# Mattdl/CLsurvey

Hardware: AMD Instinct MI355X
Metric: images/sec (train+importance pass), EWC small_VGG9 Tiny-ImageNet task batch (higher is better)
Workload: dtype f32 (bf16x6 split operands on the conv fwd/bwd-data matrix products, fp32 accumulate); 1 GPU; EWC small_VGG9_cl_128_128, Tiny-ImageNet shapes (3x64x64, 20 classes), batch 200: train step + Fisher step (BASELINE configs[1]); batch=200, parallelism=1 GPU

## Files before the change

### clsurvey_amd/_lib.py

```python
import ctypes as C
import os

_HERE = os.path.dirname(os.path.abspath(__file__))
LIB_PATH = os.path.join(_HERE, "libclhip.so")

_p = C.c_void_p
_i = C.c_int
_f = C.c_float
_z = C.c_size_t
_l = C.c_long


class HatParam(C.Structure):
    _fields_ = [("theta", _p), ("grad", _p), ("buf", _p), ("mask_back", _p), ("n", _z), ("is_emb", _i), ("reserved", _i)]


class HatGateJob(C.Structure):
    _fields_ = [("emb_row", _p), ("gate", _p), ("mask_pre", _p), ("n", _i), ("reserved", _i)]


class HatLayer(C.Structure):
    _fields_ = [("w", _p), ("gate_in", _p), ("out", _p), ("K", _z), ("C", _z), ("R", _z)]


class HatWgradJob(C.Structure):
    _fields_ = [("g", _p), ("w", _p), ("gate_in", _p), ("dgate_in", _p), ("K", _i), ("C", _i), ("R", _i), ("reserved", _i)]


class HatEmbJob(C.Structure):
    _fields_ = [("dgate", _p), ("gate", _p), ("mask_pre", _p), ("demb", _p), ("n", _i), ("rows", _i), ("t", _i), ("reserved", _i)]


class PathnetLayer(C.Structure):
    _fields_ = [("w_off", _l), ("b_off", _l), ("pw_off", _l), ("pb_off", _l), ("mod_stride", _l), ("c_out", _i), ("c_in", _i),
                ("R", _i), ("n_out", _i), ("n_in", _i), ("Kp", _i), ("Cp", _i), ("M", _i), ("path", _i * 8),
                ("trainable", C.c_ulonglong)]


class IcarlClass(C.Structure):
    _fields_ = [("row_begin", _i), ("row_end", _i), ("k", _i), ("out_off", _i)]


class LayerDesc(C.Structure):
    _fields_ = [("type", _i), ("cin", _i), ("cout", _i), ("relu", _i), ("pool", _i),
                ("w_off", _l), ("b_off", _l), ("ksize", _i), ("stride", _i), ("pad", _i), ("pool_k", _i), ("pool_s", _i),
                ("bn", _i), ("bn_w_off", _l), ("bn_b_off", _l), ("has_drop", _i)]


SIGNATURES = {
    "clhip_version": (_i, []),
    "clhip_arch": (C.c_char_p, []),
    "clhip_conv3x3_fwd": (_i, [_p, _p, _p, _p, _i, _i, _i, _i, _i, _i, _p]),
    "clhip_conv3x3_relu_pool_fwd": (_i, [_p, _p, _p, _p, _p, _i, _i, _i, _i, _i, _p]),
    "clhip_conv3x3_bwd_weight_unpool": (_i, [_p, _p, _p, _p, _p, _i, _i, _i, _i, _i, _p, _z, _p]),
    "clhip_conv3x3_bwd_data": (_i, [_p, _p, _p, _p, _i, _i, _i, _i, _i, _p]),
    "clhip_conv3x3_bwd_data_unpool": (_i, [_p, _p, _p, _p, _p, _i, _i, _i, _i, _i, _p]),
    "clhip_conv3x3_bwd_weight_ws": (_z, [_i, _i, _i, _i, _i]),
    "clhip_conv3x3_bwd_weight": (_i, [_p, _p, _p, _p, _i, _i, _i, _i, _i, _p, _z, _p]),
    "clhip_conv3x3_bwd_weight_slabs": (_i, [_p, _p, _p, _i, _i, _i, _i, _i, _p, _z, C.POINTER(_i), _p]),
    "clhip_conv3x3_bwd_weight_reduce": (_i, [_p, _p, _p, _i, _i, _i, _p]),
    "clhip_conv3x3_wino_ws": (_z, [_i, _i]),
    "clhip_conv3x3_wino_fwd": (_i, [_p, _p, _p, _p, _p, _i, _i, _i, _i, _i, _i, _p, _z, _p]),
    "clhip_conv3x3_wino_bwd_data": (_i, [_p, _p, _p, _p, _p, _i, _i, _i, _i, _i, _p, _z, _p]),
    "clhip_conv5x5_bs_ws": (_z, [_i, _i]),
    "clhip_conv5x5_bs_fwd": (_i, [_p, _p, _p, _p, _i, _i, _i, _i, _i, _i, _p, _z, _p]),
    "clhip_conv5x5_bs_bwd_data": (_i, [_p, _p, _p, _p, _i, _i, _i, _i, _i, _p, _z, _p]),
    "clhip_conv3x3_bs_ws": (_z, [_i, _i]),
    "clhip_conv3x3_bs_fwd": (_i, [_p, _p, _p, _p, _p, _i, _i, _i, _i, _i, _i, _p, _z, _p]),
    "clhip_conv3x3_bs_bwd_data": (_i, [_p, _p, _p, _p, _p, _i, _i, _i, _i, _i, _p, _z, _p]),
    "clhip_conv3x3_wino_bwd_weight_ws": (_z, [_i, _i, _i, _i, _i]),
    "clhip_conv3x3_wino_bwd_weight": (_i, [_p, _p, _p, _p, _p, _i, _i, _i, _i, _i, _p, _z, _p]),
    "clhip_conv3x3_wino_bwd_ws": (_z, [_i, _i, _i, _i, _i]),
    "clhip_conv3x3_wino_bwd": (_i, [_p, _p, _p, _p, _p, _p, _p, _p, _i, _i, _i, _i, _i, _p, _z, _p]),
    "clhip_maxpool2_fwd": (_i, [_p, _p, _p, _i, _i, _i, _p]),
    "clhip_maxpool2_bwd": (_i, [_p, _p, _p, _i, _i, _i, _p]),
    "clhip_fc_ws": (_z, [_i, _i, _i]),
    "clhip_fc_fwd": (_i, [_p, _p, _p, _p, _i, _i, _i, _i, _p, _z, _p]),
    "clhip_fc_bwd_data": (_i, [_p, _p, _p, _p, _i, _i, _i, _p, _z, _p]),
    "clhip_fc_bwd_weight": (_i, [_p, _p, _p, _p, _i, _i, _i, _p, _z, _p]),
    "clhip_relu_bwd": (_i, [_p, _p, _p, _z, _p]),
    "clhip_softmax_ce": (_i, [_p, _p, _i, _i, _i, _p, _p, _p, _p]),
    "clhip_mse_zero_sum": (_i, [_p, _z, _p, _p, _p]),
    "clhip_reg_sgd_step": (_i, [_p, _p, _p, _p, _p, _z, _f, _f, _f, _f, _i, _p]),
    "clhip_fisher_accum": (_i, [_p, _p, _z, _f, _p]),
    "clhip_mas_accum": (_i, [_p, _p, _z, _f, _f, _p]),
    "clhip_si_step": (_i, [_p, _p, _p, _p, _p, _p, _z, _f, _f, _f, _f, _i, _p]),
    "clhip_si_consolidate": (_i, [_p, _p, _p, _p, _z, _f, _p]),
    "clhip_maxpool_fwd": (_i, [_p, _p, _p, _i, _i, _i, _i, _i, _p]),
    "clhip_maxpool_bwd": (_i, [_p, _p, _p, _i, _i, _i, _i, _i, _p]),
    "clhip_conv2d_bwd_weight_ws": (_z, [_i] * 9),
    "clhip_conv2d_fwd": (_i, [_p, _p, _p, _p] + [_i] * 10 + [_p]),
    "clhip_conv2d_bwd_data": (_i, [_p, _p, _p, _p] + [_i] * 9 + [_p]),
    "clhip_conv2d_bwd_weight": (_i, [_p, _p, _p, _p] + [_i] * 9 + [_p, _z, _p]),
    "clhip_conv3x3_bs_bwd_weight_ws": (_z, [_i] * 5),
    "clhip_conv3x3_bs_bwd_weight": (_i, [_p] * 5 + [_i] * 5 + [_p, _z, _p]),
    "clhip_conv5x5_bs_bwd_weight_ws": (_z, [_i] * 5),
    "clhip_conv5x5_bs_bwd_weight": (_i, [_p] * 4 + [_i] * 5 + [_p, _z, _p]),
    "clhip_conv2d_s2d_ws": (_z, [_i] * 8),
    "clhip_conv2d_s2d_fwd": (_i, [_p, _p, _p, _p] + [_i] * 9 + [_p, _z, _p]),
    "clhip_conv2d_s2d_bwd_weight": (_i, [_p, _p, _p, _p] + [_i] * 8 + [_p, _z, _p]),
    "clhip_imm_merge": (_i, [_p, _p, _p, _i, _z, _p, _p]),
    "clhip_lwf_loss": (_i, [_p, _p, _p, _p, _i, _i, _i, _i, _f, _f, _i, _p, _p, _p, _p]),
    "clhip_packnet_finetune_mask": (_i, [_p, _z, _i, _p]),
    "clhip_packnet_kth_ws": (_z, []),
    "clhip_packnet_kth_abs": (_i, [_p, _p, _z, _i, _z, _p, _p, _z, _p]),
    "clhip_packnet_prune": (_i, [_p, _p, _z, _i, _p, _p]),
    "clhip_mask_grad_zero": (_i, [_p, _p, _z, _i, _p]),
    "clhip_mask_weight_zero": (_i, [_p, _p, _z, _i, _i, _p]),
    "clhip_packnet_sgd_step": (_i, [_p, _p, _p, _p, _z, _i, _f, _f, _f, _i, _p]),
    "clhip_hat_gate": (_i, [_p, _i, _f, _p, _p]),
    "clhip_hat_scale_weight": (_i, [_p, _p, _p, _z, _z, _z, _p]),
    "clhip_hat_weight_grad": (_i, [_p, _p, _p, _p, _p, _i, _i, _i, _p]),
    "clhip_hat_emb_grad": (_i, [_p, _p, _p, _i, _f, _f, _p, _p]),
    "clhip_hat_reg_sums": (_i, [_p, _p, _i, _p, _p]),
    "clhip_hat_backmask": (_i, [_p, _p, _p, _z, _z, _z, _p]),
    "clhip_hat_sgd_ws": (_z, []),
    "clhip_hat_sgd_step": (_i, [_p, _p, _p, _p, _z, _f, _f, _f, _i, _i, _f, _f, _f, _f, _i, _p, _z, _p]),
    "clhip_clamp": (_i, [_p, _z, _f, _f, _p]),
    "clhip_hat_sgd_multi_ws": (_z, [_i]),
    "clhip_hat_sgd_step_multi": (_i, [_p, _i, _f, _f, _f, _i, _f, _f, _f, _f, _f, _i, _p, _z, _p]),
    "clhip_hat_gates_multi": (_i, [_p, _i, _f, _p, _p]),
    "clhip_hat_scale_weights_multi": (_i, [_p, _i, _p]),
    "clhip_hat_weight_grads_multi": (_i, [_p, _i, _p]),
    "clhip_hat_emb_grads_multi": (_i, [_p, _i, _f, _f, _f, _p, _p]),
    "clhip_pathnet_ws": (_z, [_p, _i]),
    "clhip_pathnet_pack_multi": (_i, [_p, _i, _p, _z, _p, _z, _p]),
    "clhip_pathnet_fold_grads_multi": (_i, [_p, _i, _p, _z, _p, _z, _p, _z, _p]),
    "clhip_pathnet_sgd_step": (_i, [_p, _i, _p, _p, _p, _z, _f, _f, _f, _f, _i, _p, _z, _p]),
    "clhip_softmax_ce_slice": (_i, [_p, _p, _i, _i, _i, _i, _i, _p, _p, _p, _p]),
    "clhip_net_loss_step_slice": (_i, [_p, _p, _p, _p, _p, _i, _i, _i, _i, _p, _p, _p, _p, _p]),
    "clhip_axpy": (_i, [_p, _p, _z, _f, _i, _p]),
    "clhip_gem_gram_ws": (_z, [_i]),
    "clhip_gem_gram": (_i, [_p, _z, C.POINTER(_i), _i, _z, _p, _p, _z, _p]),
    "clhip_gem_project": (_i, [_p, _z, C.POINTER(_i), C.POINTER(_f), _i, _p, _p, _z, _p]),
    "clhip_gem_qp": (_i, [_p, _i, C.c_double, C.c_double, _p, _p, _p]),
    "clhip_gem_project_dev": (_i, [_p, _z, C.POINTER(_i), _p, _p, _i, _p, _p, _z, _p]),
    "clhip_gem_gram_wide_ws": (_z, [_i]),
    "clhip_gem_gram_wide": (_i, [_p, _z, C.POINTER(_i), _i, _z, _p, _p, _z, _p]),
    "clhip_gem_qp_wide_ws": (_z, [_i]),
    "clhip_gem_qp_wide": (_i, [_p, _i, C.c_double, C.c_double, _p, _p, _p, _z, _p]),
    "clhip_gem_project_wide": (_i, [_p, _z, C.POINTER(_i), C.POINTER(_f), _i, _p, _p, _z, _p]),
    "clhip_gem_project_dev_wide": (_i, [_p, _z, C.POINTER(_i), _p, _p, _i, _p, _p, _z, _p]),
    "clhip_net_create": (_i, [C.POINTER(LayerDesc), _i, _i, _i, _i, _i, C.POINTER(_p)]),
    "clhip_net_set_dropout": (_i, [_p, _i, _p, _l]),
    "clhip_net_set_bn": (_i, [_p, _i, _p, _p, _f, _f]),
    "clhip_net_set_training": (_i, [_p, _i]),
    "clhip_net_probe": (_i, [_p, _i]),
    "clhip_net_probe_read": (_i, [_p, C.POINTER(_f), C.POINTER(_i)]),
    "clhip_net_layer_input": (_i, [_p, _i, _p, _p]),
    "clhip_net_layer_pool_idx": (_i, [_p, _i, _p, _p]),
    "clhip_net_prepared_weights": (_i, [_p, _p, _p]),
    "clhip_net_edge_grid_count": (_i, [_p]),
    "clhip_net_layer_paths": (_i, [_p, _i]),
    "clhip_net_probe_kind": (_i, [_p, _i, _i]),
    "clhip_net_set_input_grad": (_i, [_p, _i, _p]),
    "clhip_sigmoid_fwd": (_i, [_p, _p, _z, _p]),
    "clhip_sigmoid_bwd": (_i, [_p, _p, _p, _z, _p]),
    "clhip_mse_mean": (_i, [_p, _p, _z, _f, _p, _p, _p]),
    "clhip_adadelta_step": (_i, [_p, _p, _p, _p, _z, _f, _f, _f, _f, _p]),
    "clhip_bn_ws": (_z, [_i]),
    "clhip_bn_fwd": (_i, [_p, _p, _p, _p, _p, _p, _p, _p, _i, _i, _i, _i, _f, _f, _i, _p, _z, _p]),
    "clhip_bn_bwd": (_i, [_p, _p, _p, _p, _p, _p, _p, _p, _p, _i, _i, _i, _i, _i, _p, _z, _p]),
    "clhip_net_destroy": (None, [_p]),
    "clhip_net_workspace_bytes": (_z, [_p]),
    "clhip_net_num_classes": (_i, [_p]),
    "clhip_net_forward": (_i, [_p, _p, _p, _i, _p, _p, _p]),
    "clhip_net_backward": (_i, [_p, _p, _p, _p, _i, _p, _p, _p]),
    "clhip_net_loss_step": (_i, [_p, _p, _p, _p, _p, _i, _i, _p, _p, _p, _p, _p]),
    "clhip_rehearsal_assemble": (_i, [_p, _p, _i, _z, _p, _p, _l, _l, _i, _p, _i, _p, _p, _p]),
    "clhip_rehearsal_assemble_crop_flip": (_i, [_p, _p, _i, _i, _i, _i, _i, _i, _p, _l, _p, _p, _p, _l, _l, _i, _p, _p, _i, _p, _p, _p]),
    "clhip_rehearsal_assemble_resized_crop_flip": (_i, [_p, _p, _i, _i, _i, _i, _i, _i, _p, _l, _p, _p, _p, _l, _l, _i, _p, _p, _i, _p, _p, _p]),
    "clhip_loss_segments": (_i, [_p, _p, _p, _i, _i, _i, _p, _i, _f, _p, _p, _p, _p]),
    "clhip_net_loss_step_loss_segments": (_i, [_p, _p, _p, _p, _p, _p, _i, _i, _p, _i, _f, _p, _p, _p, _p, _p]),
    "clhip_gather_tasks": (_i, [_p, _i, _z, _p, _i, _p, _p, _p]),
    "clhip_slice_argmax_count": (_i, [_p, _i, _i, _p, _i, _p, _p, _p, _p, _p]),
    "clhip_gather_tasks_crop_flip": (_i, [_p, _i, _i, _i, _i, _i, _i, _p, _p, _i, _p, _p, _p]),
    "clhip_gather_tasks_resized_crop_flip": (_i, [_p, _i, _i, _i, _i, _i, _i, _p, _p, _i, _p, _p, _p]),
    "clhip_gather_tasks_u8": (_i, [_p, _i, _i, _z, _p, _p, _i, _p, _p, _p]),
    "clhip_gather_tasks_crop_flip_u8": (_i, [_p, _i, _i, _i, _i, _i, _i, _p, _p, _p, _i, _p, _p, _p]),
    "clhip_gather_tasks_resized_crop_flip_u8": (_i, [_p, _i, _i, _i, _i, _i, _i, _p, _p, _p, _i, _p, _p, _p]),
    "clhip_rehearsal_assemble_crop_flip_u8": (_i, [_p, _p, _i, _i, _i, _i, _i, _i, _p, _p, _l, _p, _p, _p, _l, _l, _i, _p, _p, _i, _p, _p, _p]),
    "clhip_rehearsal_assemble_resized_crop_flip_u8": (_i, [_p, _p, _i, _i, _i, _i, _i, _i, _p, _p, _l, _p, _p, _p, _l, _l, _i, _p, _p, _i, _p, _p, _p]),
    "clhip_icarl_herd": (_i, [_p, _l, _i, _p, C.POINTER(IcarlClass), _i, _p, _l, _p]),
    "clhip_icarl_herd_wide_ws": (_z, [_i, _i]),
    "clhip_icarl_herd_wide": (_i, [_p, _l, _i, _p, C.POINTER(IcarlClass), _i, _p, _l, _p, _z, _p]),
    "clhip_icarl_nme": (_i, [_p, _p, _i, _i, _i, _i, _i, _p, _p]),
    "clhip_icarl_assemble_crop_flip": (_i, [_p, _p, _i, _i, _i, _i, _i, _i, _p, _l, _p, _p, _i, _p, _i, _p, _p, _p, _p]),
    "clhip_icarl_assemble_crop_flip_u8": (_i, [_p, _p, _i, _i, _i, _i, _i, _i, _p, _p, _l, _p, _p, _i, _p, _i, _p, _p, _p, _p]),
    "clhip_icarl_assemble_resized_crop_flip": (_i, [_p, _p, _i, _i, _i, _i, _i, _i, _p, _l, _p, _p, _i, _p, _i, _p, _p, _p, _p]),
    "clhip_icarl_assemble_resized_crop_flip_u8": (_i, [_p, _p, _i, _i, _i, _i, _i, _i, _p, _p, _l, _p, _p, _i, _p, _i, _p, _p, _p, _p]),
}

_lib = None


def lib():
    global _lib
    if _lib is None:
        path = os.environ.get("CLHIP_LIB", LIB_PATH)
        if not os.path.exists(path):
            raise RuntimeError(
                "clsurvey_amd: %s not found. Build it with `python clsurvey_amd/build.py` "
                "(hipcc --offload-arch=gfx950). There is no CPU fallback." % path)
        import torch
        bundled = os.path.join(os.path.dirname(torch.__file__), "lib", "libamdhip64.so")
        if os.path.exists(bundled):
            C.CDLL(bundled, mode=C.RTLD_GLOBAL)
        h = C.CDLL(path)
        for name, (res, args) in SIGNATURES.items():
            fn = getattr(h, name)
            fn.restype = res
            fn.argtypes = args
        _lib = h
    return _lib


class ClhipError(RuntimeError):
    pass


def check(rc, what):
    if rc != 0:
        if rc > 0:
            raise ClhipError("%s: HIP error %d" % (what, rc))
        names = {-1: "CLHIP_EINVAL", -2: "CLHIP_ENOSPC", -3: "CLHIP_ENOTSUP"}
        raise ClhipError("%s: %s" % (what, names.get(rc, rc)))
```

### clsurvey_amd/csrc/bsconv.hip

```cpp
#include "common.hpp"
#include "bs_weight.hpp"
#include <cstdlib>

#ifndef BS_ABL
#define BS_ABL 0
#endif

namespace {

constexpr int BS_WT_JOBS = 24;
struct BsWtJobs { int n; int pad; clhip_wino_wt j[BS_WT_JOBS]; int first[BS_WT_JOBS + 1]; };

__global__ __launch_bounds__(256) void bs_weight_multi_kernel(BsWtJobs J) {
    int jb = 0;
    for (int i = 1; i < J.n; ++i) jb = ((int)blockIdx.x >= J.first[i]) ? i : jb;
    bs_weight_block(J.j[jb], (int)blockIdx.x - J.first[jb], (int)threadIdx.x);
}

template <int RW_, int RH_, int NI_, int WAVES_M_, int WM_, int WN_, int KS_ = 3>
struct BsGeo {
    static constexpr int RW = RW_, RH = RH_, NI = NI_, WAVES_M = WAVES_M_, WAVES_N = 4 / WAVES_M_, WM = WM_, WN = WN_;
    static constexpr int KS = KS_, HP = KS_ / 2, TAPS = KS_ * KS_;
    static constexpr int BM = RW * RH * NI;
    static_assert(BM == 32 * WAVES_M * WM, "pixels per block = M tiles of the waves");
    static_assert(32 * WAVES_N * WN == BS_BN, "64 output channels per block");
    static constexpr int MTW = RW >= 16 ? 16 : 8, MTH = 32 / MTW;
    static_assert(RW % MTW == 0 && RH % MTH == 0, "whole M tiles");
    static constexpr int MT_PER_ROW = RW / MTW, MT_PER_IMG = MT_PER_ROW * (RH / MTH);
    static constexpr int IPR = RW == 8 ? 2 : 1;
    static_assert(NI % IPR == 0, "image pairs");
    static constexpr int HW_ = RW + 2 * HP, HR = RH + 2 * HP;
    static constexpr int P = (IPR * HW_ + 7) / 16 * 16 + 8;
    static_assert(P >= IPR * HW_ && P % 16 == 8, "pitch");
    static constexpr int ROWS = (NI / IPR) * HR;
    static constexpr int PLANE_SLOTS = (ROWS - 1) * P + IPR * HW_;
    static constexpr int PLANE_BYTES = PLANE_SLOTS * 16;
    static constexpr int BUF_BYTES = 6 * PLANE_BYTES;
    static constexpr int NHALO = NI * HR * HW_;
    static constexpr int ITEMS = 2 * NHALO;
    static constexpr int ROUNDS = (ITEMS + 255) / 256;
    static_assert(ROUNDS * 256 - ITEMS <= ITEMS, "the last round wraps at most once");
    static constexpr int TPR = WM < MT_PER_ROW ? WM : MT_PER_ROW;
    static_assert(WM % TPR == 0 && MT_PER_ROW % TPR == 0 && MT_PER_IMG % WM == 0, "a wave's tiles form a rectangle inside one image");
    static constexpr int RGW = TPR * MTW, RGH = 32 * WM / RGW;
    static constexpr int TS = 32 * WM + 4;
    static_assert(4 * 32 * TS * 4 <= 2 * BUF_BYTES, "transposition buffers fit the staging LDS");
};

template <class G, int MODE, bool UNPOOL>
__device__ __forceinline__ void bs_conv_body(
    unsigned char* __restrict__ lds, const int b, const float* __restrict__ in, const clhip_u32x4* __restrict__ wimg,
    const float* __restrict__ bias, const float* __restrict__ mask_src, float* __restrict__ out, uint8_t* __restrict__ pool_idx, int N,
    int Cin, int Cout, int H, int W, int relu, int tiles_x, int tiles_y, int npb) {
    constexpr int RW = G::RW, RH = G::RH, NI = G::NI, WM = G::WM, WN = G::WN, P = G::P, HR = G::HR, HW_ = G::HW_;
    constexpr int ROUNDS = G::ROUNDS;

    const int tid = threadIdx.x, lane = tid & 63, wave = tid >> 6;
    const int kts = (Cout + BS_BN - 1) / BS_BN;
    const int kt = (b >> 3) % kts, pb = (b / (8 * kts)) * 8 + (b & 7);
    if (pb >= npb) return;
    const int tx = pb % tiles_x, ty = (pb / tiles_x) % tiles_y, grp = pb / (tiles_x * tiles_y);
    const int n0 = grp * NI, y0 = ty * RH, x0 = tx * RW;
    const int n_chunks = Cin / BS_CK;
    const int IH = UNPOOL ? H >> 1 : H, IW = UNPOOL ? W >> 1 : W;
    const int plane_in = IH * IW;

    const float* in_blk = in + (size_t)n0 * Cin * plane_in;
    const __amdgpu_buffer_rsrc_t rs_x = clhip_rsrc(in_blk, (size_t)(N - n0) * Cin * plane_in * sizeof(float));
    const __amdgpu_buffer_rsrc_t rs_i = clhip_rsrc(UNPOOL ? pool_idx + (size_t)n0 * Cin * plane_in : pool_idx,
                                                   UNPOOL ? (size_t)(N - n0) * Cin * plane_in : 0);
    const int n_nt = (Cout + 31) / 32;
    constexpr int TAPS = G::TAPS, KS = G::KS;
    const __amdgpu_buffer_rsrc_t rs_w = clhip_rsrc(wimg, (size_t)n_nt * n_chunks * 3 * TAPS * 1024);

    int xoff[ROUNDS], lw[ROUNDS], pos[ROUNDS];
#pragma unroll
    for (int r = 0; r < ROUNDS; ++r) {
        const int it_ = r * 256 + tid, it = it_ < G::ITEMS ? it_ : it_ - G::ITEMS;
        const int h = it >= G::NHALO ? 1 : 0, p = it - h * G::NHALO;
        const int ni = p / (HR * HW_), rem = p - ni * (HR * HW_), hy = rem / HW_, hx = rem - hy * HW_;
        const int gy = y0 + hy - G::HP, gx = x0 + hx - G::HP, n = n0 + ni;
        const bool ok = n < N && gy >= 0 && gy < H && gx >= 0 && gx < W;
        const int e = UNPOOL ? (gy >> 1) * IW + (gx >> 1) : gy * IW + gx;
        xoff[r] = ok ? (ni * Cin + 8 * h) * plane_in + e : CLHIP_OOB;
// ... 238 lines not shown
                if (MODE == 0) {
                    y00 += bv; y01 += bv; y10 += bv; y11 += bv;
                    if (relu) { y00 = fmaxf(y00, 0.f); y01 = fmaxf(y01, 0.f); y10 = fmaxf(y10, 0.f); y11 = fmaxf(y11, 0.f); }
                    if (pool) {
                        float mx = y00; int am = 0;
                        if (y01 > mx) { mx = y01; am = 1; }
                        if (y10 > mx) { mx = y10; am = 2; }
                        if (y11 > mx) { mx = y11; am = 3; }
                        if (relu && !(mx > 0.f)) am = CLHIP_POOL_DEAD;
                        if (ok && (!(BS_ABL & 16) || mx == 12345.678f)) {
                            const size_t o = ((size_t)n * Cout + k) * OH * OW + (size_t)(oh >> 1) * OW + (ow >> 1);
                            out[o] = mx;
                            pool_idx[o] = (uint8_t)am;
                        }
                        continue;
                    }
                }
                if (!ok || ((BS_ABL & 16) && y00 != 12345.678f)) continue;
                const size_t o = ((size_t)n * Cout + k) * chw + (size_t)oh * W + ow;
                if (odd) {
                    const bool row1 = oh + 1 < H, col1 = ow + 1 < W;
                    if (MODE == 1 && mask_src) {
                        y00 = mask_src[o] > 0.f ? y00 : 0.f;
                        if (col1) y01 = mask_src[o + 1] > 0.f ? y01 : 0.f;
                        if (row1) y10 = mask_src[o + W] > 0.f ? y10 : 0.f;
                        if (row1 && col1) y11 = mask_src[o + W + 1] > 0.f ? y11 : 0.f;
                    }
                    out[o] = y00;
                    if (col1) out[o + 1] = y01;
                    if (row1) out[o + W] = y10;
                    if (row1 && col1) out[o + W + 1] = y11;
                } else {
                    if (MODE == 1 && mask_src) {
                        const float2 m0 = *reinterpret_cast<const float2*>(mask_src + o), m1 = *reinterpret_cast<const float2*>(mask_src + o + W);
                        y00 = m0.x > 0.f ? y00 : 0.f; y01 = m0.y > 0.f ? y01 : 0.f;
                        y10 = m1.x > 0.f ? y10 : 0.f; y11 = m1.y > 0.f ? y11 : 0.f;
                    }
                    *reinterpret_cast<float2*>(out + o) = make_float2(y00, y01);
                    *reinterpret_cast<float2*>(out + o + W) = make_float2(y10, y11);
                }
            }
        }
    }
    }
}

template <class G, bool UNPOOL>
constexpr int bs_blocks_per_cu() {
    return (3 * 2 * G::BUF_BYTES <= 160 * 1024 && (G::RW == 32 || (!UNPOOL && G::KS == 3))) ? 3 : 2;
}

template <class G, int MODE, bool UNPOOL>
__global__ __launch_bounds__(256, (bs_blocks_per_cu<G, UNPOOL>())) void bs_conv_kernel(
    const float* __restrict__ in, const clhip_u32x4* __restrict__ wimg, const float* __restrict__ bias,
    const float* __restrict__ mask_src, float* __restrict__ out, uint8_t* __restrict__ pool_idx, int N, int Cin, int Cout, int H,
    int W, int relu, int tiles_x, int tiles_y, int npb) {
    __shared__ __attribute__((aligned(16))) unsigned char lds[2 * G::BUF_BYTES];
    bs_conv_body<G, MODE, UNPOOL>(lds, (int)blockIdx.x, in, wimg, bias, mask_src, out, pool_idx, N, Cin, Cout, H, W, relu, tiles_x, tiles_y, npb);
}

template <class GA, class GB, int MODE, bool UNPOOL>
__global__ __launch_bounds__(256, (bs_blocks_per_cu<GA, UNPOOL>() < bs_blocks_per_cu<GB, UNPOOL>() ? bs_blocks_per_cu<GA, UNPOOL>()
                                                                                                  : bs_blocks_per_cu<GB, UNPOOL>()))
void bs_conv_mixed_kernel(const float* __restrict__ in, const clhip_u32x4* __restrict__ wimg, const float* __restrict__ bias,
                          const float* __restrict__ mask_src, float* __restrict__ out, uint8_t* __restrict__ pool_idx, int N, int Cin,
                          int Cout, int H, int W, int relu, int blocks_a, int NA, int tiles_xa, int tiles_ya, int npb_a, int tiles_xb,
                          int tiles_yb, int npb_b) {
    constexpr int LB = 2 * (GA::BUF_BYTES > GB::BUF_BYTES ? GA::BUF_BYTES : GB::BUF_BYTES);
    __shared__ __attribute__((aligned(16))) unsigned char lds[LB];
    const int b = (int)blockIdx.x;
    if (b < blocks_a) {
        bs_conv_body<GA, MODE, UNPOOL>(lds, b, in, wimg, bias, mask_src, out, pool_idx, NA, Cin, Cout, H, W, relu, tiles_xa, tiles_ya, npb_a);
    } else {
        const size_t in_img = (size_t)Cin * (UNPOOL ? (size_t)(H >> 1) * (W >> 1) : (size_t)H * W);
        const bool pool = MODE == 0 && pool_idx != nullptr;
        const size_t out_img = (size_t)Cout * (pool ? (size_t)(H >> 1) * (W >> 1) : (size_t)H * W);
        uint8_t* idx_b = pool_idx ? pool_idx + (size_t)NA * (UNPOOL ? in_img : out_img) : nullptr;
        bs_conv_body<GB, MODE, UNPOOL>(lds, b - blocks_a, in + (size_t)NA * in_img, wimg, bias,
                                       mask_src ? mask_src + (size_t)NA * Cout * H * W : nullptr, out + (size_t)NA * out_img, idx_b, N - NA,
                                       Cin, Cout, H, W, relu, tiles_xb, tiles_yb, npb_b);
    }
}


static int bs_env_int(const char* name, int dflt) {
    const char* e = getenv(name);
    return e && e[0] ? atoi(e) : dflt;
}

template <class G, int MODE, bool UNPOOL>
int bs_launch_geo(const float* in, const clhip_u32x4* wimg, const float* bias, const float* mask_src, float* out, uint8_t* pool_idx,
                  int N, int Cin, int Cout, int H, int W, int relu, hipStream_t s) {
    const int tiles_x = (W + G::RW - 1) / G::RW, tiles_y = (H + G::RH - 1) / G::RH, groups = (N + G::NI - 1) / G::NI;
    const long long npb = (long long)tiles_x * tiles_y * groups;
    const int kts = (Cout + BS_BN - 1) / BS_BN;
    const long long blocks = (npb + 7) / 8 * 8 * kts;
    if (blocks <= 0 || blocks > 0x7fffffffLL) return CLHIP_EINVAL;
    hipLaunchKernelGGL((bs_conv_kernel<G, MODE, UNPOOL>), dim3((unsigned)blocks), dim3(256), 0, s, in, wimg, bias, mask_src, out,
                       pool_idx, N, Cin, Cout, H, W, relu, tiles_x, tiles_y, (int)npb);
    CLHIP_LAUNCH_CHECK();
    return 0;
}

template <int MODE, bool UNPOOL>
int bs_launch_mixed32(const float* in, const clhip_u32x4* wimg, const float* bias, const float* mask_src, float* out, uint8_t* pool_idx,
                      int N, int Cin, int Cout, int H, int W, int relu, hipStream_t s, bool* taken) {
    using GA = BsGeo<32, 4, 1, 2, 2, 1>;
    using GB = BsGeo<32, 2, 1, 2, 1, 1>;
    *taken = false;
    static const int on = bs_env_int("CLHIP_BS_MIXED", 1);
    if (!on) return 0;
    const int kts = (Cout + BS_BN - 1) / BS_BN;
    const long long per_img_a = (long long)((W + GA::RW - 1) / GA::RW) * ((H + GA::RH - 1) / GA::RH);
    const long long slots = 256LL * bs_blocks_per_cu<GA, UNPOOL>();
    const long long total = per_img_a * N * kts, rounds = total / slots, rem = total - rounds * slots;
    if (rounds < 1 || rem == 0 || 2 * rem > slots) return 0;
    const long long na = rounds * slots / (per_img_a * kts);
    if (na < 1 || na >= N || na % 8) return 0;
    const int NA = (int)na;
    const int txa = (W + GA::RW - 1) / GA::RW, tya = (H + GA::RH - 1) / GA::RH, txb = (W + GB::RW - 1) / GB::RW, tyb = (H + GB::RH - 1) / GB::RH;
    const long long npb_a = (long long)txa * tya * NA, npb_b = (long long)txb * tyb * (N - NA);
    const long long blocks_a = (npb_a + 7) / 8 * 8 * kts, blocks_b = (npb_b + 7) / 8 * 8 * kts;
    if (blocks_a + blocks_b > 0x7fffffffLL) return 0;
    hipLaunchKernelGGL((bs_conv_mixed_kernel<GA, GB, MODE, UNPOOL>), dim3((unsigned)(blocks_a + blocks_b)), dim3(256), 0, s, in, wimg, bias,
                       mask_src, out, pool_idx, N, Cin, Cout, H, W, relu, (int)blocks_a, NA, txa, tya, (int)npb_a, txb, tyb, (int)npb_b);
    CLHIP_LAUNCH_CHECK();
    *taken = true;
    return 0;
}

template <int MODE, bool UNPOOL>
int bs_launch(const float* in, const clhip_u32x4* wimg, const float* bias, const float* mask_src, float* out, uint8_t* pool_idx,
              int N, int Cin, int Cout, int H, int W, int relu, hipStream_t s) {
    if (W > 16 && !((H | W) & 1)) {
        bool taken = false;
        const int rc = bs_launch_mixed32<MODE, UNPOOL>(in, wimg, bias, mask_src, out, pool_idx, N, Cin, Cout, H, W, relu, s, &taken);
        if (rc || taken) return rc;
    }
#define BS_GO(...) return bs_launch_geo<BsGeo<__VA_ARGS__>, MODE, UNPOOL>(in, wimg, bias, mask_src, out, pool_idx, N, Cin, Cout, H, W, relu, s)
    if (W > 16) BS_GO(32, 4, 1, 2, 2, 1);
    if (W > 8) BS_GO(16, 8, 1, 2, 2, 1);
    BS_GO(8, 8, 2, 2, 2, 1);
#undef BS_GO
}

template <int MODE>
int bs_launch5(const float* in, const clhip_u32x4* wimg, const float* bias, const float* mask_src, float* out, int N, int Cin, int Cout,
               int H, int W, int relu, hipStream_t s) {
    if (W > 16) return bs_launch_geo<BsGeo<32, 4, 1, 2, 2, 1, 5>, MODE, false>(in, wimg, bias, mask_src, out, nullptr, N, Cin, Cout, H, W, relu, s);
    return bs_launch_geo<BsGeo<16, 8, 1, 2, 2, 1, 5>, MODE, false>(in, wimg, bias, mask_src, out, nullptr, N, Cin, Cout, H, W, relu, s);
}

}

bool clhip_internal_bs_ok(int Cin, int Cout, int H, int W) {
    return Cin >= 32 && Cin % 32 == 0 && Cout >= 64 && Cout % 64 == 0 && H >= 4 && W >= 4;
}

bool clhip_internal_bs_index_ok(int Cin, int Cout, int H, int W, int ks) {
    const long long px = (long long)H * W, ni = (ks == 3 && W <= 8) ? 2 : 1;
    const long long img = (long long)((Cout + 31) / 32) * ((Cin + BS_CK - 1) / BS_CK) * 3 * ks * ks * 1024;
    return ni * Cin * px < (1LL << 29) && Cout * px < (1LL << 29) && img <= 0x7fffffffLL;
}

bool clhip_internal_bs_preferred(int Cin, int Cout, int H, int W) {
    static const int mode = bs_env_int("CLHIP_BS", 1);
    if (mode == 0 || !clhip_internal_bs_ok(Cin, Cout, H, W)) return false;
    if (mode == 2) return true;
    const long long px = (long long)H * W;
    return (px >= 1024 && px <= 4096 && Cin <= 128 && Cout <= 128) || (px >= 512 && px < 1024 && Cin >= 256 && Cout >= 256);
}
bool clhip_internal_bs5_preferred(int Cin, int Cout, int H, int W) {
    static const int mode = bs_env_int("CLHIP_BS", 1);
    return mode != 0 && clhip_internal_bs_ok(Cin, Cout, H, W) && W > 8;
}

size_t clhip_internal_bs_ws(int Cin, int Cout) {
    return (size_t)((Cout + 31) / 32) * ((Cin + BS_CK - 1) / BS_CK) * 27 * 1024;
}
size_t clhip_internal_bs5_ws(int Cin, int Cout) {
    return (size_t)((Cout + 31) / 32) * ((Cin + BS_CK - 1) / BS_CK) * 75 * 1024;
}

int clhip_internal_bs_weights(const clhip_wino_wt* jobs, int n, hipStream_t s) {
    if (n <= 0) return 0;
    if (!jobs) return CLHIP_EINVAL;
    for (int base = 0; base < n; base += BS_WT_JOBS) {
        BsWtJobs J;
        J.n = n - base < BS_WT_JOBS ? n - base : BS_WT_JOBS;
        J.pad = 0;
        int blocks = 0;
        for (int i = 0; i < J.n; ++i) {
            const clhip_wino_wt& q = jobs[base + i];
            if (!q.w || !q.U || q.Ko <= 0 || q.Ci <= 0) return CLHIP_EINVAL;
            J.j[i] = q;
            J.first[i] = blocks;
            blocks += bs_weight_blocks(q);
        }
        J.first[J.n] = blocks;
        hipLaunchKernelGGL(bs_weight_multi_kernel, dim3(blocks), dim3(256), 0, s, J);
        CLHIP_LAUNCH_CHECK();
    }
    return 0;
}

int clhip_internal_bs_conv_u(int mode, const float* in, const void* wimg, const float* bias, const float* mask_src, float* out,
                             uint8_t* pool_idx, int unpool, int N, int Cin, int Cout, int H, int W, int relu, hipStream_t s) {
    if (!in || !wimg || !out || N <= 0 || !clhip_internal_bs_ok(Cin, Cout, H, W) || !clhip_internal_bs_index_ok(Cin, Cout, H, W, 3)) return CLHIP_EINVAL;
    if (((H | W) & 1) && (pool_idx || unpool)) return CLHIP_ENOTSUP;
    const clhip_u32x4* img = static_cast<const clhip_u32x4*>(wimg);
    if (mode == 0) return bs_launch<0, false>(in, img, bias, nullptr, out, pool_idx, N, Cin, Cout, H, W, relu, s);
    if (unpool) return bs_launch<1, true>(in, img, nullptr, mask_src, out, pool_idx, N, Cin, Cout, H, W, 0, s);
    return bs_launch<1, false>(in, img, nullptr, mask_src, out, nullptr, N, Cin, Cout, H, W, 0, s);
}

int clhip_internal_bs5_conv_u(int mode, const float* in, const void* wimg, const float* bias, const float* mask_src, float* out, int N,
                              int Cin, int Cout, int H, int W, int relu, hipStream_t s) {
    if (!in || !wimg || !out || N <= 0 || !clhip_internal_bs_ok(Cin, Cout, H, W) || W <= 8 || !clhip_internal_bs_index_ok(Cin, Cout, H, W, 5))
        return CLHIP_EINVAL;
    const clhip_u32x4* img = static_cast<const clhip_u32x4*>(wimg);
    if (mode == 0) return bs_launch5<0>(in, img, bias, nullptr, out, N, Cin, Cout, H, W, relu, s);
    return bs_launch5<1>(in, img, nullptr, mask_src, out, N, Cin, Cout, H, W, 0, s);
}

extern "C" {

size_t clhip_conv5x5_bs_ws(int C, int K) {
    const size_t a = clhip_internal_bs5_ws(C, K), b = clhip_internal_bs5_ws(K, C);
    return a > b ? a : b;
}

int clhip_conv5x5_bs_fwd(const float* x, const float* w, const float* b, float* y, int N, int C, int K, int H, int W, int relu, void* ws,
                         size_t ws_bytes, void* stream) {
    if (N <= 0 || !clhip_internal_bs_ok(C, K, H, W) || W <= 8) return CLHIP_ENOTSUP;
    if (!x || !w || !y || !ws || ws_bytes < clhip_internal_bs5_ws(C, K)) return CLHIP_EINVAL;
    if (!clhip_internal_bs_index_ok(C, K, H, W, 5)) return CLHIP_EINVAL;
    const clhip_wino_wt job{w, static_cast<float*>(ws), K, C, 0, 5};
    const int rc = clhip_internal_bs_weights(&job, 1, as_stream(stream));
    if (rc) return rc;
    return clhip_internal_bs5_conv_u(0, x, ws, b, nullptr, y, N, C, K, H, W, relu, as_stream(stream));
}

int clhip_conv5x5_bs_bwd_data(const float* dy, const float* w, const float* relu_src, float* dx, int N, int C, int K, int H, int W,
                              void* ws, size_t ws_bytes, void* stream) {
    if (N <= 0 || !clhip_internal_bs_ok(K, C, H, W) || W <= 8) return CLHIP_ENOTSUP;
    if (!dy || !w || !dx || !ws || ws_bytes < clhip_internal_bs5_ws(K, C)) return CLHIP_EINVAL;
    if (!clhip_internal_bs_index_ok(K, C, H, W, 5)) return CLHIP_EINVAL;
    const clhip_wino_wt job{w, static_cast<float*>(ws), C, K, 1, 5};
    const int rc = clhip_internal_bs_weights(&job, 1, as_stream(stream));
    if (rc) return rc;
    return clhip_internal_bs5_conv_u(1, dy, ws, nullptr, relu_src, dx, N, K, C, H, W, 0, as_stream(stream));
}

size_t clhip_conv3x3_bs_ws(int C, int K) {
    const size_t a = clhip_internal_bs_ws(C, K), b = clhip_internal_bs_ws(K, C);
    return a > b ? a : b;
}

int clhip_conv3x3_bs_fwd(const float* x, const float* w, const float* b, float* y, uint8_t* idx_u8_or_null, int N, int C, int K, int H,
                         int W, int relu, void* ws, size_t ws_bytes, void* stream) {
    if (N <= 0 || !clhip_internal_bs_ok(C, K, H, W)) return CLHIP_ENOTSUP;
    if (!x || !w || !y || !ws || ws_bytes < clhip_internal_bs_ws(C, K)) return CLHIP_EINVAL;
    if (!clhip_internal_bs_index_ok(C, K, H, W, 3)) return CLHIP_EINVAL;
    if (((H | W) & 1) && idx_u8_or_null) return CLHIP_ENOTSUP;
    const clhip_wino_wt job{w, static_cast<float*>(ws), K, C, 0, 0};
    const int rc = clhip_internal_bs_weights(&job, 1, as_stream(stream));
    if (rc) return rc;
    return clhip_internal_bs_conv_u(0, x, ws, b, nullptr, y, idx_u8_or_null, 0, N, C, K, H, W, relu, as_stream(stream));
}

int clhip_conv3x3_bs_bwd_data(const float* dy, const uint8_t* idx_u8_or_null, const float* w, const float* relu_src, float* dx, int N,
                              int C, int K, int H, int W, void* ws, size_t ws_bytes, void* stream) {
    if (N <= 0 || !clhip_internal_bs_ok(K, C, H, W)) return CLHIP_ENOTSUP;
    if (!dy || !w || !dx || !ws || ws_bytes < clhip_internal_bs_ws(K, C)) return CLHIP_EINVAL;
    if (!clhip_internal_bs_index_ok(K, C, H, W, 3)) return CLHIP_EINVAL;
    if (((H | W) & 1) && idx_u8_or_null) return CLHIP_ENOTSUP;
    const clhip_wino_wt job{w, static_cast<float*>(ws), C, K, 1, 0};
    const int rc = clhip_internal_bs_weights(&job, 1, as_stream(stream));
    if (rc) return rc;
    return clhip_internal_bs_conv_u(1, dy, ws, nullptr, relu_src, dx, const_cast<uint8_t*>(idx_u8_or_null), idx_u8_or_null != nullptr,
                                    N, K, C, H, W, 0, as_stream(stream));
}

}
```

### clsurvey_amd/csrc/common.hpp

```cpp
#pragma once
#include <hip/hip_runtime.h>
#include <stdint.h>
#include <stddef.h>
#include "../../include/clhip.h"

#define CLHIP_LAUNCH_CHECK()                          \
    do {                                              \
        hipError_t e__ = hipGetLastError();           \
        if (e__ != hipSuccess) return (int)e__;       \
    } while (0)

static inline hipStream_t as_stream(void* s) { return reinterpret_cast<hipStream_t>(s); }

static inline bool aligned16(const void* p) { return (reinterpret_cast<uintptr_t>(p) & 15u) == 0; }

static inline bool clhip_conv3x3_dims_ok(int N, int C, int K, int H, int W) {
    if (N <= 0 || C <= 0 || K <= 0 || H <= 0 || W <= 0) return false;
    const long long hw = (long long)H * W;
    if (hw >= (1LL << 23)) return false;
    if (hw * (C + 32LL) >= (1LL << 28) || hw * (K + 32LL) >= (1LL << 28)) return false;
    if ((long long)K * C >= (1LL << 29) / 9) return false;
    return hw * N <= 0x7fffffffLL;
}

// ... 60 lines not shown
    return v;
}
__device__ __forceinline__ float wave_sum(float v) {
#pragma unroll
    for (int o = 32; o > 0; o >>= 1) v += __shfl_xor(v, o, 64);
    return v;
}
__device__ __forceinline__ double wave_sum(double v) {
#pragma unroll
    for (int o = 32; o > 0; o >>= 1) v += __shfl_xor(v, o, 64);
    return v;
}
__device__ __forceinline__ int wave_min(int v) {
#pragma unroll
    for (int o = 32; o > 0; o >>= 1) v = min(v, __shfl_xor(v, o, 64));
    return v;
}

typedef float floatx16 __attribute__((ext_vector_type(16)));
typedef float floatx4 __attribute__((ext_vector_type(4)));

__device__ __forceinline__ int mfma32_row(int r, int lane) { return (r & 3) + 8 * (r >> 2) + 4 * (lane >> 5); }


#define CLHIP_FC_MAX 4
struct clhip_fc_chain {
    int n;
    long w_off[CLHIP_FC_MAX], b_off[CLHIP_FC_MAX];
    int din[CLHIP_FC_MAX], dout[CLHIP_FC_MAX], relu[CLHIP_FC_MAX];
    size_t act_off[CLHIP_FC_MAX], dz_off[CLHIP_FC_MAX];
};
int clhip_internal_fc_chain_ok(const clhip_fc_chain* d);
int clhip_internal_fc_chain_wgrad(const clhip_fc_chain* d, float* grads, const float* x, int N, const float* acts,
                                  const float* dlogits, const float* dz, hipStream_t s);
struct clhip_gemm_args {
    const float* a; const float* b; float* out;
    int M, N, K; long sam, sak, sbk, sbn; int n_tiles, splits, k_per_split;
    const float* bias; const float* mask_src; int relu;
};
int clhip_internal_fc_bwd_data_args(const float* dy, const float* w, const float* relu_src, float* dx, int M, int I, int O,
                                    clhip_gemm_args* args_out);
int clhip_internal_fc_bwd_combo(const clhip_gemm_args* g, int gemm_blocks, const clhip_fc_chain* d, float* grads, const float* x,
                                int N, const float* acts, const float* dlogits, const float* dz, hipStream_t s);

int clhip_internal_fc_tail_ok(const clhip_fc_chain* d);
int clhip_internal_fc_tail(const clhip_fc_chain* d, const float* params, float* acts, int N, const int64_t* labels,
                           int reduction, int col_off, int ncols, float* dlogits, float* fcdz, float* loss_out, double* stats,
                           void* row_scratch, unsigned* counter, int do_loss, int do_bwd, const float* h1_slabs, int live,
                           hipStream_t s);
int clhip_internal_fc_fwd_partial(const float* x, const float* w, int M, int I, int O, void* ws, size_t ws_bytes, int* live,
                                  hipStream_t s);

#define CLHIP_WGRAD_JOBS_MAX 32
struct clhip_wgrad_job { const float* part; float* dw; float* db; int K, C, splits; int taps; };
int clhip_internal_conv3x3_wgrad_partial(const float* x, const float* dy, const uint8_t* unpool_idx, float* dw, float* db, int N,
                                         int C, int K, int H, int W, void* ws, size_t ws_bytes, void* stream, clhip_wgrad_job* job);
int clhip_internal_wgrad_reduce_multi(const clhip_wgrad_job* jobs, int n, hipStream_t s);

bool clhip_internal_convkk_ok(int N, int Cin, int Cout, int H, int W, int R, int S, int stride, int pad);
int clhip_internal_convkk(int mode, const float* in, const float* w, const float* bias, const float* mask_src, float* out, int N,
                          int Cin, int Cout, int H, int W, int relu, hipStream_t s);

struct clhip_wino_wt { const float* w; float* U; int Ko, Ci, mode, pad; };
int clhip_internal_wino_weights(const clhip_wino_wt* jobs, int n, hipStream_t s);
int clhip_internal_weight_images(const clhip_wino_wt* wino_jobs, int n_wino, const clhip_wino_wt* bs_jobs, int n_bs, hipStream_t s);
int clhip_internal_c3w64_pool_weight_images(const float* x, const float* w, const float* b, float* y_pool, uint8_t* idx_u8, int N, int C,
                                            int K, int H, int W, const clhip_wino_wt* wino_jobs, int n_wino, const clhip_wino_wt* bs_jobs,
                                            int n_bs, int wt_first, hipStream_t s);
int clhip_internal_wino_conv_u(int mode, const float* in, const float* U, const float* bias, const float* mask_src, float* out,
                               uint8_t* pool_idx, int unpool, int N, int Cin, int Cout, int H, int W, int relu, hipStream_t s);
bool clhip_internal_wino_ok(int Cin, int Cout, int H, int W);
size_t clhip_internal_wino_ws(int Cin, int Cout);
bool clhip_internal_bs_ok(int Cin, int Cout, int H, int W);
bool clhip_internal_bs_index_ok(int Cin, int Cout, int H, int W, int ks);
bool clhip_internal_bs_preferred(int Cin, int Cout, int H, int W);
bool clhip_internal_bs5_preferred(int Cin, int Cout, int H, int W);
size_t clhip_internal_bs5_ws(int Cin, int Cout);
int clhip_internal_bs5_conv_u(int mode, const float* in, const void* wimg, const float* bias, const float* mask_src, float* out, int N,
                              int Cin, int Cout, int H, int W, int relu, hipStream_t s);
size_t clhip_internal_bs_ws(int Cin, int Cout);
int clhip_internal_bs_weights(const clhip_wino_wt* jobs, int n, hipStream_t s);
int clhip_internal_bs_conv_u(int mode, const float* in, const void* wimg, const float* bias, const float* mask_src, float* out,
                             uint8_t* pool_idx, int unpool, int N, int Cin, int Cout, int H, int W, int relu, hipStream_t s);
bool clhip_internal_bs5_wgrad_ok(int N, int C, int K, int H, int W);
size_t clhip_internal_bs5_wgrad_ws(int N, int C, int K, int H, int W);
int clhip_internal_bs5_wgrad(const float* x, const float* dy, float* dw, float* db, int N, int C, int K, int H, int W, void* ws,
                             size_t ws_bytes, hipStream_t s);
size_t clhip_internal_bs3k_wgrad_ws(int N, int C, int K, int H, int W);
int clhip_internal_bs3k_wgrad(const float* x, const float* dy, float* dw, float* db, int N, int C, int K, int H, int W, void* ws,
                              size_t ws_bytes, hipStream_t s);
bool clhip_internal_bs_wgrad_ok(int C, int K, int H, int W);
bool clhip_internal_bs_wgrad_preferred(int C, int K, int H, int W, int pooled);
size_t clhip_internal_bs_wgrad_ws(int N, int C, int K, int H, int W);
int clhip_internal_bs_wgrad_partial(const float* x, const float* dy, const uint8_t* unpool_idx, float* dw, float* db, int N, int C, int K,
                                    int H, int W, void* ws, size_t ws_bytes, hipStream_t s, clhip_wgrad_job* job);
bool clhip_internal_wino_wgrad_ok(int C, int K, int H, int W);
size_t clhip_internal_wino_wgrad_ws(int N, int C, int K, int H, int W);
int clhip_internal_wino_wgrad_partial(const float* x, const float* dy, const uint8_t* unpool_idx, float* dw, float* db, int N, int C,
                                      int K, int H, int W, void* ws, size_t ws_bytes, hipStream_t s, clhip_wgrad_job* job);
int clhip_internal_wino_pair(const float* dy, const uint8_t* unpool_idx, const float* U, const float* mask_src, float* dx,
                             const float* x, float* dw, float* db, int N, int C, int K, int H, int W, void* ws, size_t ws_bytes,
                             hipStream_t s, clhip_wgrad_job* job);
bool clhip_internal_wino_pair_shape(int N, int C, int K, int H, int W, int pooled);
int clhip_internal_wino_conv(int mode, const float* in, const float* w, const float* bias, const float* mask_src, float* out,
                             uint8_t* pool_idx, int unpool, int N, int Cin, int Cout, int H, int W, int relu, void* ws,
                             size_t ws_bytes, hipStream_t s);
```

### clsurvey_amd/csrc/conv3x3_wgrad.hip

```cpp
#include <cstdlib>
#include "common.hpp"

namespace {

constexpr int KT = 64, CT = 64;

#ifdef CLHIP_TRACE
__device__ unsigned long long* g_wtrace = nullptr;
#define TR_NOW() __builtin_amdgcn_s_memtime()
#endif

template <int TW, int TH>
struct WGeo {
    static constexpr int BP = TW * TH;
    static constexpr int TWP = TW + 2;
    static constexpr int PLANE = (TH + 2) * TWP;
    static constexpr int PLANEP = PLANE | 1;
    static constexpr int LDP = BP + 1;
    static_assert(BP == 64, "stage is 64 pixels");
};

__device__ __forceinline__ void decode_stage(int st, int tiles_w, int tiles_h, int TW, int TH,
                                             int& n, int& h0, int& w0) {
    int tw_i = st % tiles_w;
    int t = st / tiles_w;
    int th_i = t % tiles_h;
    n = t / tiles_h;
    h0 = th_i * TH;
    w0 = tw_i * TW;
}

#ifndef CLHIP_WGRAD_PS_WAVES
#define CLHIP_WGRAD_PS_WAVES 1
#endif
template <int TW, int TH, bool VEC, bool PS, bool UNPOOL = false>
__global__ __launch_bounds__(256, CLHIP_WGRAD_PS_WAVES) void conv3x3_wgrad_kernel(
    const float* __restrict__ x, const float* __restrict__ dy, float* __restrict__ part,
    int N, int C, int K, int H, int W, int tiles_w, int tiles_h,
    int total_stages, int splits, int c_tiles, size_t slab_stride, const uint8_t* __restrict__ unpool_idx) {
    static_assert(!UNPOOL || VEC, "the fused un-pool lives in the 16-byte staging path");
    using G = WGeo<TW, TH>;
    constexpr int KTt = PS ? 32 : 64, CTt = PS ? 32 : 64;
    constexpr int DYS_FLOATS = KTt * G::LDP, XS_FLOATS = CTt * G::PLANEP;
    constexpr int BUF_FLOATS = DYS_FLOATS + XS_FLOATS;
    static_assert(!PS || 2 * BUF_FLOATS >= 9 * 1024 + 3 * 128, "the pixel-split reduction pad lives in the stage buffers");
    __shared__ __attribute__((aligned(16))) float lds[2 * BUF_FLOATS];

    const int tid = threadIdx.x, lane = tid & 63, wave = tid >> 6;
#ifdef CLHIP_TRACE
    const unsigned long long tr_start = TR_NOW();
#endif
    const int wk = PS ? 0 : (wave & 1), wc = PS ? 0 : (wave >> 1);
    const int li = lane & 31, kk = lane >> 5;

    const int split = blockIdx.x % splits;
    const int tile = blockIdx.x / splits;
    const int ct = tile % c_tiles, kt = tile / c_tiles;
    const int k0 = kt * KTt, c0 = ct * CTt;

    const int per = total_stages / splits, extra = total_stages % splits;
    const int st_begin = split * per + min(split, extra);
    const int st_end = st_begin + per + (split < extra ? 1 : 0);

    floatx16 acc[9];
#pragma unroll
    for (int t = 0; t < 9; ++t)
#pragma unroll
        for (int r = 0; r < 16; ++r) acc[t][r] = 0.f;
    double bsum = 0.0;

    const int plane_hw = H * W;
    const int Wp = W >> 1, plane_dy = UNPOOL ? (H >> 1) * Wp : plane_hw;

    constexpr int XROWS = CTt * (TH + 2);
    constexpr int DY_IT = VEC ? (KTt * G::BP / 4) / 256 : KTt * G::BP / 256;
    constexpr int X_ELEMS = CTt * G::PLANE;
    constexpr int XV_ELEMS = XROWS * (TW / 4);
    constexpr int X_IT = VEC ? (XV_ELEMS + 255) / 256 : (X_ELEMS + 255) / 256;
    constexpr int H_IT = VEC ? (XROWS * 2 + 255) / 256 : 0;
    constexpr int NU = DY_IT + X_IT + H_IT;
    float4 dyv[VEC ? DY_IT : 1], xv[VEC ? X_IT : 1];
    float hv[H_IT > 0 ? H_IT : 1];
    float dyr[VEC ? 1 : DY_IT], xr[VEC ? 1 : X_IT];
    int dyoff[DY_IT], dydst[DY_IT], dyrow[DY_IT];
// ... 526 lines not shown
        cur_n = t0 / tiles_h;
    }
    auto load_stage = [&](Stage& S, bool live) {
        const int n = cur_n, h0 = cur_th * 2, w0 = cur_tw * 32;
        if (++cur_tw == tiles_w) { cur_tw = 0; if (++cur_th == tiles_h) { cur_th = 0; ++cur_n; } }
        const int o = __builtin_amdgcn_readfirstlane(live ? (n * K * OH + (h0 >> 1)) * OW + (w0 >> 1) : 0);
        S.gA = clhip_buf_load4(r_dy, live ? dyA_voff : CLHIP_OOB, o * 4);
        S.gB = clhip_buf_load4(r_dy, live ? dyB_voff : CLHIP_OOB, o * 4);
        S.code8 = clhip_buf_load2(r_ix, live ? ix8_voff : CLHIP_OOB, o);
        const int hrow = h0 + wh;
        const unsigned edges = (hrow == 0 ? 1u : 0u) | (hrow + 1 >= H ? 2u : 0u) | (w0 == 0 ? 4u : 0u) | (w0 + 32 >= W ? 8u : 0u);
        const unsigned bad = live ? edge_bits & (unsigned)__builtin_amdgcn_readfirstlane((int)(edges * 0x11111u)) : 0xfffffu;
        const int xo = __builtin_amdgcn_readfirstlane(live ? ((n * C * H + hrow) * W + w0) * 4 : 0);
#pragma unroll
        for (int j = 0; j < 5; ++j)
            S.xr[j] = clhip_buf_load(r_x, (bad & (0xfu << (4 * j))) ? CLHIP_OOB : xe_voff[j], xo);
    };
    auto store_x = [&](const Stage& S, int buf) {
        float* d = xs_w + buf * U3_HALO;
#pragma unroll
        for (int j = 0; j < 5; ++j) d[xe_dst[j]] = S.xr[j];
        float* dd = dy_w + buf * U3_DY;
        *reinterpret_cast<float4*>(dd + dstA) = S.gA;
        *reinterpret_cast<float4*>(dd + dstB) = S.gB;
        *reinterpret_cast<float2*>(dd + dst8) = S.code8;
    };
    auto compute = [&](int buf) {
        const float* row = dy_w + buf * U3_DY + li * U3_DYROW;
        float4 Sg[4];
#pragma unroll
        for (int j = 0; j < 4; ++j) Sg[j] = *reinterpret_cast<const float4*>(row + 4 * j);
        const clhip_u32x4 Scode = *reinterpret_cast<const clhip_u32x4*>(row + 16);
        const float* bp = xs_w + buf * U3_HALO + col_off + kk;
        asm volatile("" : "+a"(acc));
#pragma unroll
        for (int wp = 0; wp < 16; ++wp) {
            const float g = wp & 2 ? (wp & 1 ? Sg[wp >> 2].w : Sg[wp >> 2].z) : (wp & 1 ? Sg[wp >> 2].y : Sg[wp >> 2].x);
            const unsigned word = Scode[wp >> 2];
            const unsigned code = (word >> (8 * (wp & 3))) & 0xffu;
            const float a = code == want ? g : 0.f;
            bsum += (double)a;
            acc = __builtin_amdgcn_mfma_f32_32x32x2f32(a, bp[2 * wp], acc, 0, 0, 0);
        }
        asm volatile("" : "+a"(acc));
    };

    const int n_st = st_end - st_begin;
    if (n_st > 0) {
        Stage SA, SB;
        load_stage(SA, true);
        store_x(SA, 0);
        const int pairs = n_st >> 1;
        for (int i = 0; i < pairs; ++i) {
            load_stage(SB, true);
            compute(0);
            store_x(SB, 1);
            load_stage(SA, 2 * i + 2 < n_st);
            compute(1);
            store_x(SA, 0);
        }
        if (n_st & 1) compute(0);
    }
    bsum += __shfl_xor(bsum, 32, 64);
    if (wh == 1) {
#pragma unroll
        for (int r = 0; r < 16; ++r) red[(wk * 16 + r) * 64 + lane] = acc[r];
        if (kk == 0) red[2048 + wk * 32 + li] = (float)bsum;
    }
    __syncthreads();
    if (wh == 0) {
        float* slab = part + (size_t)split * slab_stride;
        if (li < ncol) {
            const int cc = li / 9, rs = li - cc * 9;
#pragma unroll
            for (int r = 0; r < 16; ++r) {
                const int kr = k0 + wk * 32 + mfma32_row(r, lane);
                if (kr < K) slab[((size_t)rs * K + kr) * C + cc] = acc[r] + red[(wk * 16 + r) * 64 + lane];
            }
        }
        if (kk == 0 && kok) slab[(size_t)9 * K * C + k] = (float)(bsum + (double)red[2048 + wk * 32 + li]);
    }
}

constexpr int RED_EL = 64, RED_J = 16, RED_V = 4;
constexpr int RED_THREADS = RED_EL / RED_V * RED_J;

template <int EL, int J>
__device__ __forceinline__ void wgrad_reduce_block(const float* __restrict__ part, float* __restrict__ dw, float* __restrict__ db,
                                                   int K, int C, int splits, size_t e0, double (*partial)[EL], int T = 9) {
    const size_t kc = (size_t)K * C, nw = (size_t)T * kc, total = nw + K;
    const int v = threadIdx.x % (EL / RED_V), j = threadIdx.x / (EL / RED_V);
    const size_t e = e0 + (size_t)v * RED_V;
    const int q = (splits + J - 1) / J;
    const int s0 = j * q, s1 = min(splits, s0 + q);
    double s[RED_V] = {0.0, 0.0, 0.0, 0.0};
    if ((total & 3) == 0 && (reinterpret_cast<uintptr_t>(part) & 15u) == 0 && e + RED_V <= total) {
#pragma unroll 4
        for (int sp = s0; sp < s1; ++sp) {
            const float4 t = *reinterpret_cast<const float4*>(part + (size_t)sp * total + e);
            s[0] += (double)t.x; s[1] += (double)t.y; s[2] += (double)t.z; s[3] += (double)t.w;
        }
    } else {
        for (int sp = s0; sp < s1; ++sp)
#pragma unroll
            for (int t = 0; t < RED_V; ++t)
                if (e + t < total) s[t] += (double)part[(size_t)sp * total + e + t];
    }
#pragma unroll
    for (int t = 0; t < RED_V; ++t) partial[j][v * RED_V + t] = s[t];
    __syncthreads();
    if (threadIdx.x < EL) {
        const int el = threadIdx.x;
        const size_t ee = e0 + el;
        if (ee < total) {
            double t = 0.0;
#pragma unroll
            for (int jj = 0; jj < J; ++jj) t += partial[jj][el];
            if (ee < nw) {
                const size_t rs = ee / kc, rem = ee - rs * kc;
                dw[rem * T + rs] = (float)t;
            } else if (db) {
                db[ee - nw] = (float)t;
            }
        }
    }
}

template <int EL, int J>
__global__ __launch_bounds__(RED_THREADS) void wgrad_reduce_kernel(const float* __restrict__ part, float* __restrict__ dw,
                                                                   float* __restrict__ db, int K, int C, int splits) {
    __shared__ double partial[J][EL];
    wgrad_reduce_block<EL, J>(part, dw, db, K, C, splits, (size_t)blockIdx.x * EL, partial);
}

struct RedJobs {
    clhip_wgrad_job job[CLHIP_WGRAD_JOBS_MAX];
    unsigned first[CLHIP_WGRAD_JOBS_MAX + 1];
    int n;
};

template <int EL, int JL>
__global__ __launch_bounds__(RED_THREADS) void wgrad_reduce_multi_kernel(RedJobs jobs) {
    __shared__ double partial[JL][EL];
    int ji = 0;
    while (ji + 1 < jobs.n && blockIdx.x >= jobs.first[ji + 1]) ++ji;
    const clhip_wgrad_job J = jobs.job[ji];
    wgrad_reduce_block<EL, JL>(J.part, J.dw, J.db, J.K, J.C, J.splits, (size_t)(blockIdx.x - jobs.first[ji]) * EL, partial, J.taps ? J.taps : 9);
}

struct WPlan {
    int TW, TH, tiles_w, tiles_h, total_stages, splits, k_tiles, c_tiles, group, groups, ps;
    size_t slab, ws_floats;
};

WPlan make_plan(int N, int C, int K, int H, int W) {
    WPlan p;
    if (W > 16) { p.TW = 32; p.TH = 2; }
    else if (W > 8) { p.TW = 16; p.TH = 4; }
    else { p.TW = 8; p.TH = 8; }
    p.tiles_w = (W + p.TW - 1) / p.TW;
    p.tiles_h = (H + p.TH - 1) / p.TH;
    p.total_stages = p.tiles_w * p.tiles_h * N;
    const bool smallc = (C * 9 <= 32);
    p.k_tiles = (K + KT - 1) / KT;
    p.c_tiles = smallc ? 1 : (C + CT - 1) / CT;
    p.ps = 0;
    if (!smallc) {
        const int t64 = p.k_tiles * p.c_tiles;
        const int splits64 = (256 + t64 - 1) / t64;
        if (p.total_stages / (splits64 > 0 ? splits64 : 1) < 8) {
            p.ps = 1;
            p.k_tiles = (K + 31) / 32;
            p.c_tiles = (C + 31) / 32;
        }
    }
    int tiles = p.k_tiles * p.c_tiles;
    int target = smallc ? 1024 : 256;
    if (smallc) {
        static const int t_env = [] { const char* e = getenv("CLHIP_WG_SMALLC_BLOCKS"); return e && e[0] ? atoi(e) : 0; }();
        if (t_env > 0) target = t_env;
    }
    int splits = (target + tiles - 1) / tiles;
    if (splits > p.total_stages) splits = p.total_stages;
    p.slab = (size_t)9 * K * C + K;
    size_t max_splits = ((size_t)64 << 20) / (p.slab * sizeof(float));
    if (max_splits < 1) max_splits = 1;
    if ((size_t)splits > max_splits) splits = (int)max_splits;
    if (splits < 1) splits = 1;
    p.splits = splits;
    int group = 1;
    while (group * group < splits) ++group;
    p.group = group;
    p.groups = (splits + group - 1) / group;
    p.ws_floats = p.slab * (size_t)(splits + p.groups);
    return p;
}

}

extern "C" {

#ifdef CLHIP_TRACE
int clhip_debug_set_wgrad_trace(void* p) {
    unsigned long long* q = static_cast<unsigned long long*>(p);
    return (int)hipMemcpyToSymbol(HIP_SYMBOL(g_wtrace), &q, sizeof(q));
}
#endif

size_t clhip_conv3x3_bwd_weight_ws(int N, int C, int K, int H, int W) {
    if (!clhip_conv3x3_dims_ok(N, C, K, H, W)) return 0;
    return make_plan(N, C, K, H, W).ws_floats * sizeof(float);
}

static int bwd_weight_impl(const float* x, const float* dy, const uint8_t* unpool_idx, float* dw, float* db,
                           int N, int C, int K, int H, int W, void* ws, size_t ws_bytes, void* stream,
                           clhip_wgrad_job* defer = nullptr) {
    if (!x || !dy || !dw || !ws || !clhip_conv3x3_dims_ok(N, C, K, H, W)) return CLHIP_EINVAL;
    if (unpool_idx && ((H & 1) || (W & 1))) return CLHIP_ENOTSUP;
    WPlan p = make_plan(N, C, K, H, W);
    if (ws_bytes < p.ws_floats * sizeof(float)) return CLHIP_ENOSPC;
    hipStream_t s = as_stream(stream);
    float* part = static_cast<float*>(ws);
    const bool smallc = (C * 9 <= 32);
    unsigned grid = (unsigned)(p.k_tiles * p.c_tiles * p.splits);
#define WG_ARGS x, dy, part, N, C, K, H, W, p.tiles_w, p.tiles_h, p.total_stages, p.splits
    if (smallc && unpool_idx && p.TW == 32 && W % 32 == 0 && aligned16(dy) && aligned16(unpool_idx) &&
        (size_t)N * K * H * W < ((size_t)1 << 31) && (size_t)N * C * H * W < ((size_t)1 << 29)) {
        hipLaunchKernelGGL(conv3x3_wgrad_c3_unpool_kernel, dim3(grid), dim3(256), 0, s, WG_ARGS, p.slab, unpool_idx);
    } else if (smallc) {
        if (p.TW == 32) hipLaunchKernelGGL((conv3x3_wgrad_smallc_kernel<32, 2>), dim3(grid), dim3(256), 0, s, WG_ARGS, p.slab, unpool_idx);
        else if (p.TW == 16) hipLaunchKernelGGL((conv3x3_wgrad_smallc_kernel<16, 4>), dim3(grid), dim3(256), 0, s, WG_ARGS, p.slab, unpool_idx);
        else hipLaunchKernelGGL((conv3x3_wgrad_smallc_kernel<8, 8>), dim3(grid), dim3(256), 0, s, WG_ARGS, p.slab, unpool_idx);
    } else {
        const bool vec = (W % 4 == 0) && (W % p.TW == 0) && aligned16(x) && aligned16(dy);
        if (unpool_idx && (!vec || (reinterpret_cast<uintptr_t>(unpool_idx) & 1u))) return CLHIP_ENOTSUP;
#define WG_K(TW_, TH_, VEC_, PS_, UNP_) hipLaunchKernelGGL((conv3x3_wgrad_kernel<TW_, TH_, VEC_, PS_, UNP_>), dim3(grid), dim3(256), 0, s, \
                                                           WG_ARGS, p.c_tiles, p.slab, unpool_idx)
#define WG_LAUNCH1(TW_, TH_, PS_) do { if (unpool_idx) WG_K(TW_, TH_, true, PS_, true); else if (vec) WG_K(TW_, TH_, true, PS_, false); \
                                      else WG_K(TW_, TH_, false, PS_, false); } while (0)
#define WG_LAUNCH(TW_, TH_) do { if (p.ps) WG_LAUNCH1(TW_, TH_, true); else WG_LAUNCH1(TW_, TH_, false); } while (0)
        if (p.TW == 32) WG_LAUNCH(32, 2);
        else if (p.TW == 16) WG_LAUNCH(16, 4);
        else WG_LAUNCH(8, 8);
#undef WG_LAUNCH
#undef WG_LAUNCH1
#undef WG_K
    }
#undef WG_ARGS
    CLHIP_LAUNCH_CHECK();
    if (defer) {
        *defer = clhip_wgrad_job{part, dw, db, K, C, p.splits};
        return 0;
    }
    const unsigned bx = (unsigned)((p.slab + RED_EL - 1) / RED_EL);
    hipLaunchKernelGGL((wgrad_reduce_kernel<RED_EL, RED_J>), dim3(bx), dim3(RED_THREADS), 0, s, part, dw, db, K, C, p.splits);
    CLHIP_LAUNCH_CHECK();
    return 0;
}

int clhip_conv3x3_bwd_weight(const float* x, const float* dy, float* dw, float* db,
                             int N, int C, int K, int H, int W, void* ws, size_t ws_bytes, void* stream) {
    return bwd_weight_impl(x, dy, nullptr, dw, db, N, C, K, H, W, ws, ws_bytes, stream);
}

int clhip_conv3x3_bwd_weight_unpool(const float* x, const float* dy_pool, const uint8_t* idx_u8, float* dw, float* db,
                                    int N, int C, int K, int H, int W, void* ws, size_t ws_bytes, void* stream) {
    if (!idx_u8) return CLHIP_EINVAL;
    return bwd_weight_impl(x, dy_pool, idx_u8, dw, db, N, C, K, H, W, ws, ws_bytes, stream);
}

int clhip_conv3x3_bwd_weight_slabs(const float* x, const float* dy, const uint8_t* idx_u8_or_null, int N, int C, int K, int H,
                                   int W, void* ws, size_t ws_bytes, int* splits_out, void* stream) {
    if (!splits_out || !ws) return CLHIP_EINVAL;
    clhip_wgrad_job job;
    const int rc = bwd_weight_impl(x, dy, idx_u8_or_null, static_cast<float*>(ws), nullptr, N, C, K, H, W, ws, ws_bytes, stream, &job);
    if (rc == 0) *splits_out = job.splits;
    return rc;
}

int clhip_conv3x3_bwd_weight_reduce(const void* ws, float* dw, float* db, int K, int C, int splits, void* stream) {
    if (!ws || !dw || K <= 0 || C <= 0 || splits <= 0) return CLHIP_EINVAL;
    const size_t slab = (size_t)9 * K * C + K;
    const unsigned bx = (unsigned)((slab + RED_EL - 1) / RED_EL);
    hipLaunchKernelGGL((wgrad_reduce_kernel<RED_EL, RED_J>), dim3(bx), dim3(RED_THREADS), 0, as_stream(stream),
                            static_cast<const float*>(ws), dw, db, K, C, splits);
    CLHIP_LAUNCH_CHECK();
    return 0;
}

}

int clhip_internal_conv3x3_wgrad_partial(const float* x, const float* dy, const uint8_t* unpool_idx, float* dw, float* db, int N,
                                         int C, int K, int H, int W, void* ws, size_t ws_bytes, void* stream, clhip_wgrad_job* job) {
    if (!job) return CLHIP_EINVAL;
    return bwd_weight_impl(x, dy, unpool_idx, dw, db, N, C, K, H, W, ws, ws_bytes, stream, job);
}

int clhip_internal_wgrad_reduce_multi(const clhip_wgrad_job* jobs, int n, hipStream_t s) {
    if (n <= 0) return 0;
    if (!jobs || n > CLHIP_WGRAD_JOBS_MAX) return CLHIP_EINVAL;
    RedJobs r;
    r.n = n;
    r.first[0] = 0;
    for (int i = 0; i < n; ++i) {
        r.job[i] = jobs[i];
        const size_t total = (size_t)(jobs[i].taps ? jobs[i].taps : 9) * jobs[i].K * jobs[i].C + jobs[i].K;
        r.first[i + 1] = r.first[i] + (unsigned)((total + RED_EL - 1) / RED_EL);
    }
    for (int i = n; i < CLHIP_WGRAD_JOBS_MAX; ++i) { r.job[i] = clhip_wgrad_job{nullptr, nullptr, nullptr, 0, 0, 0, 0}; r.first[i + 1] = r.first[n]; }
    hipLaunchKernelGGL((wgrad_reduce_multi_kernel<RED_EL, RED_J>), dim3(r.first[n]), dim3(RED_THREADS), 0, s, r);
    CLHIP_LAUNCH_CHECK();
    return 0;
}
```

### clsurvey_amd/csrc/engine.hip

```cpp
#include <vector>
#include <cstdlib>
#include <memory>
#include <new>
#include "common.hpp"

namespace {

enum class Conv : unsigned char {
    None,
    Direct3,
    Wino,
    Bs3,
    Bs5,
    S2d,
    Gemm,
};
enum class Img : unsigned char { None, WinoU, Bs3, Bs5 };
struct WeightImage { Img kind; size_t off; };
enum : unsigned {
    WG_BS = 1,
    WG_WINO = 2,
    WG_3X3 = 4,
    WG_BS5 = 8,
    WG_S2D = 16,
};

struct LayerPlan {
    int type;
    int cin, cout, relu, pool;
    long w_off, b_off;
    int h, w;
    int ks, st, pd;
    int oh, ow;
    int pk, ps;
    int ph, pw;
    bool vgg;
    bool pool22;
    bool fused_pool;
    size_t in_elems, out_elems, pool_elems;
    size_t act_off;
    size_t pool_off;
    size_t idx_off;
    int bn;
    long bn_w_off, bn_b_off;
    size_t z_off;
    size_t stat_off;
    float* rmean; float* rvar; float bn_momentum, bn_eps;
    Conv fwd, bwd;
    WeightImage img_f, img_d;
    unsigned wg;
    size_t wg_off, wg_bytes;
    size_t s2d_off, s2d_bytes;
    size_t scratch_need;
    const float* extra_grad;
    const float* drop;
    long drop_stride;
    int has_drop_buf;
    size_t drop_off;
};

constexpr long long WINO_MIN_UNITS = 640;
constexpr long long WINO16_MIN_UNITS = 384;
constexpr unsigned PROBE_RING = 64;
#ifndef CLHIP_EDGE_GRIDS_DEFAULT
#define CLHIP_EDGE_GRIDS_DEFAULT 1
#endif
#ifndef CLHIP_OVERLAP_DEFAULT
#define CLHIP_OVERLAP_DEFAULT 0
#endif

bool env_starts(const char* name, char c) { const char* e = std::getenv(name); return e && e[0] == c; }
bool wino_enabled() { return !env_starts("CLHIP_WINO", '0'); }
bool bs5_wgrad_enabled() { return !env_starts("CLHIP_BS_WGRAD", '0'); }
bool s2d_enabled() { return env_starts("CLHIP_S2D", '1'); }
bool fc_tail_enabled() { return !env_starts("CLHIP_FC_TAIL", '0'); }
int overlap_mode() { return env_starts("CLHIP_WGRAD_OVERLAP", '1') ? 1 : env_starts("CLHIP_WGRAD_OVERLAP", '2') ? 2 : CLHIP_OVERLAP_DEFAULT; }
int edge_grids_mode() {
    const char* e = std::getenv("CLHIP_EDGE_GRIDS");
    return (e && e[0] >= '0' && e[0] <= '2' && !e[1]) ? e[0] - '0' : CLHIP_EDGE_GRIDS_DEFAULT;
}

struct NetPlan {
    std::vector<LayerPlan> layers;
    int max_batch, in_c, in_h, in_w, n_classes;
    size_t in_elems;
    size_t scratch_bytes;
    size_t wino_bytes;
    size_t off_wino;
    size_t off_s2d;
    int s2d_fresh_n;
    size_t total_bytes;
    size_t off_acts, off_idx, off_g0, off_g1, off_scratch, off_dlogits, off_loss, off_fcdz, off_wg;
    int training = 1;
    int n_wg;
    int fc_first;
    bool fc_fused;
    clhip_fc_chain chain;
    size_t fcdz_floats;
    int probe_layer = -1;
    int probe_kind;
    unsigned probe_count;
    std::vector<hipEvent_t> probe_ev;
    bool fc_tail, no_combo;
    unsigned* tail_counter;
    size_t off_rows;
    int edge_grids;
    unsigned edge_count;
    bool overlap;
    int overlap_mode;
    hipStream_t side;
    std::vector<hipEvent_t> ev_dy, ev_wg;
    ~NetPlan() {
        for (hipEvent_t e : ev_dy) (void)hipEventDestroy(e);
        for (hipEvent_t e : ev_wg) (void)hipEventDestroy(e);
        if (side) (void)hipStreamDestroy(side);
        if (tail_counter) (void)hipFree(tail_counter);
        for (hipEvent_t e : probe_ev) (void)hipEventDestroy(e);
    }
};

inline size_t align_up(size_t v, size_t a) { return (v + a - 1) / a * a; }
inline size_t max_of(size_t a, size_t b) { return a > b ? a : b; }

__global__ void drop_scale_kernel(float* __restrict__ h, const float* __restrict__ mask, long stride, int feat, size_t total) {
    for (size_t i = blockIdx.x * (size_t)blockDim.x + threadIdx.x; i < total; i += (size_t)gridDim.x * blockDim.x) {
        const size_t n = i / feat, f = i - n * feat;
        h[i] *= mask[n * stride + f];
    }
}

__global__ void add_inplace_kernel(float* __restrict__ a, const float* __restrict__ b, size_t n) {
    for (size_t i = blockIdx.x * (size_t)blockDim.x + threadIdx.x; i < n; i += (size_t)gridDim.x * blockDim.x) a[i] += b[i];
}

int add_inplace(float* a, const float* b, size_t n, hipStream_t s) {
    hipLaunchKernelGGL(add_inplace_kernel, dim3(ew_grid(n, 256)), dim3(256), 0, s, a, b, n);
    CLHIP_LAUNCH_CHECK();
    return 0;
}

__global__ void drop_copy_kernel(const float* __restrict__ h, float* __restrict__ out, const float* __restrict__ mask, long stride,
                                 int feat, size_t total) {
    for (size_t i = blockIdx.x * (size_t)blockDim.x + threadIdx.x; i < total; i += (size_t)gridDim.x * blockDim.x) {
        const size_t n = i / feat, f = i - n * feat;
        out[i] = h[i] * mask[n * stride + f];
    }
}

int drop_copy(const float* h, float* out, const float* mask, long stride, size_t feat, int N, hipStream_t s) {
    const size_t total = feat * N;
    hipLaunchKernelGGL(drop_copy_kernel, dim3(ew_grid(total, 256)), dim3(256), 0, s, h, out, mask, stride, (int)feat, total);
    CLHIP_LAUNCH_CHECK();
    return 0;
}

int drop_scale(float* h, const float* mask, long stride, size_t feat, int N, hipStream_t s) {
    const size_t total = feat * N;
    hipLaunchKernelGGL(drop_scale_kernel, dim3(ew_grid(total, 256)), dim3(256), 0, s, h, mask, stride, (int)feat, total);
    CLHIP_LAUNCH_CHECK();
    return 0;
}

int plan_geometry(NetPlan& p, const clhip_layer_desc* descs, int n_layers) {
    int c = p.in_c, h = p.in_h, w = p.in_w;
    size_t feat = p.in_elems;
    bool seen_fc = false;
    for (int i = 0; i < n_layers; ++i) {
        const clhip_layer_desc& d = descs[i];
        LayerPlan L{};
        L.type = d.type; L.cin = d.cin; L.cout = d.cout; L.relu = d.relu; L.pool = d.pool; L.w_off = d.w_off; L.b_off = d.b_off;
        if (L.type == 0) {
            if (seen_fc || L.cin != c) return CLHIP_EINVAL;
            L.h = h; L.w = w;
            L.ks = d.ksize > 0 ? d.ksize : 3;
            L.st = d.ksize > 0 ? d.stride : 1;
            L.pd = d.ksize > 0 ? d.pad : 1;
            if (L.st < 1 || L.pd < 0) return CLHIP_EINVAL;
            L.oh = (h + 2 * L.pd - L.ks) / L.st + 1; L.ow = (w + 2 * L.pd - L.ks) / L.st + 1;
            if (L.oh <= 0 || L.ow <= 0) return CLHIP_EINVAL;
            L.vgg = L.ks == 3 && L.st == 1 && L.pd == 1;
            L.in_elems = (size_t)c * h * w;
            L.out_elems = (size_t)L.cout * L.oh * L.ow;
            L.bn = d.bn ? 1 : 0; L.bn_w_off = d.bn_w_off; L.bn_b_off = d.bn_b_off;
            L.bn_momentum = 0.1f; L.bn_eps = 1e-5f;
            h = L.oh; w = L.ow;
            if (L.pool) {
                L.pk = d.pool_k > 0 ? d.pool_k : 2;
                L.ps = d.pool_k > 0 ? d.pool_s : 2;
                L.pool22 = L.pk == 2 && L.ps == 2;
                if (L.ps < 1 || h < L.pk || w < L.pk) return CLHIP_EINVAL;
// ... 70 lines not shown
         : kind == Img::Bs5 ? clhip_internal_bs5_ws(cin, cout) : 0;
}

void plan_classifier(NetPlan& p) {
    const int n_layers = (int)p.layers.size();
    p.fc_first = n_layers;
    for (int i = 0; i < n_layers; ++i) if (p.layers[i].type == 1) { p.fc_first = i; break; }
    const int nfc = n_layers - p.fc_first;
    if (nfc < 1 || nfc > CLHIP_FC_MAX) return;
    clhip_fc_chain& ch = p.chain;
    ch.n = nfc;
    size_t dzf = 0;
    for (int l = 0; l < nfc; ++l) {
        const LayerPlan& L = p.layers[p.fc_first + l];
        ch.w_off[l] = L.w_off; ch.b_off[l] = L.b_off; ch.din[l] = L.cin; ch.dout[l] = L.cout; ch.relu[l] = L.relu;
        ch.act_off[l] = L.act_off;
        ch.dz_off[l] = dzf;
        if (l < nfc - 1) dzf += (size_t)L.cout * p.max_batch;
    }
    p.fcdz_floats = dzf;
    p.fc_fused = clhip_internal_fc_chain_ok(&ch) != 0;
}

void layout_arena(NetPlan& p) {
    const size_t N = p.max_batch;
    size_t acts = 0, idxb = 0, gmax = 0, scratch = 0, imgs = 0, wg_total = 0, s2d_total = 0;
    for (LayerPlan& L : p.layers) {
        if (L.bn) {
            L.z_off = acts; acts += L.out_elems * N;
            L.stat_off = acts; acts += align_up(2 * (size_t)L.cout, 4);
        }
        L.act_off = acts; acts += L.out_elems * N;
        if (L.type == 0 && L.pool) {
            L.pool_off = acts; acts += L.pool_elems * N;
            L.idx_off = idxb; idxb += align_up(L.pool_elems * N, 256);
        }
        if (L.has_drop_buf) { L.drop_off = acts; acts += L.in_elems * N; }
        if (L.wg & (WG_3X3 | WG_WINO)) { L.wg_off = wg_total; wg_total += L.wg_bytes; ++p.n_wg; }
        if (L.img_f.kind != Img::None) { L.img_f.off = imgs; imgs += align_up(image_bytes(L.img_f.kind, L.cin, L.cout), 256); }
        if (L.img_d.kind != Img::None) { L.img_d.off = imgs; imgs += align_up(image_bytes(L.img_d.kind, L.cout, L.cin), 256); }
        if (L.fwd == Conv::S2d) { L.s2d_off = s2d_total; s2d_total += L.s2d_bytes; }
        scratch = max_of(scratch, L.scratch_need);
        gmax = max_of(gmax, max_of(L.in_elems, L.out_elems));
    }
    p.scratch_bytes = scratch; p.wino_bytes = imgs;
    plan_classifier(p);
    size_t off = 0;
    p.off_acts = off; off += align_up(acts * 4, 256);
    p.off_idx = off; off += align_up(idxb, 256);
    p.off_g0 = off; off += align_up(gmax * N * 4, 256);
    p.off_g1 = off; off += align_up(gmax * N * 4, 256);
    p.off_scratch = off; off += align_up(scratch, 256);
    p.off_wino = off; off += align_up(imgs, 256);
    p.off_dlogits = off; off += align_up(N * p.n_classes * 4, 256);
    p.off_loss = off; off += 256;
    p.off_fcdz = off;
    if (p.fc_fused) {
        off += align_up(p.fcdz_floats * 4 + 256, 256);
        p.off_rows = off;
        off += align_up(N * 8, 256);
    }
    p.off_wg = off;
    if (p.n_wg < 2 || p.n_wg > CLHIP_WGRAD_JOBS_MAX) p.n_wg = 0;
    if (p.n_wg) off += align_up(wg_total, 256);
    p.off_s2d = off; off += s2d_total;
    p.total_bytes = off;
}

void make_resources(NetPlan& p) {
    const size_t n_layers = p.layers.size();
    bool any_bn = false;
    for (const LayerPlan& L : p.layers) any_bn = any_bn || L.bn;
    p.overlap_mode = overlap_mode();
    if (p.overlap_mode && !any_bn) {
        if (hipStreamCreateWithFlags(&p.side, hipStreamNonBlocking) == hipSuccess) {
            p.overlap = true;
            p.ev_dy.resize(n_layers); p.ev_wg.resize(n_layers);
            for (size_t i = 0; i < n_layers && p.overlap; ++i)
                if (hipEventCreateWithFlags(&p.ev_dy[i], hipEventDisableTiming) != hipSuccess ||
                    hipEventCreateWithFlags(&p.ev_wg[i], hipEventDisableTiming) != hipSuccess) p.overlap = false;
        } else { (void)hipGetLastError(); p.side = nullptr; }
    }
    p.edge_grids = edge_grids_mode();
    const bool tail = fc_tail_enabled();
    p.no_combo = !tail;
    if (p.fc_fused && tail && clhip_internal_fc_tail_ok(&p.chain) && p.max_batch <= 1024) {
        if (hipMalloc(reinterpret_cast<void**>(&p.tail_counter), 256) == hipSuccess &&
            hipMemset(p.tail_counter, 0, 256) == hipSuccess) {
            p.fc_tail = true;
        } else {
            (void)hipGetLastError();
            if (p.tail_counter) { (void)hipFree(p.tail_counter); p.tail_counter = nullptr; }
        }
    }
}

static bool tail_usable(const NetPlan* p, const float* params, const void* ws, int N) {
    if (!p->fc_tail) return false;
    for (size_t i = p->fc_first + 1; i < p->layers.size(); ++i)
        if (p->layers[i].drop || p->layers[i].extra_grad) return false;
    const float* acts = reinterpret_cast<const float*>(static_cast<const char*>(ws) + p->off_acts);
    return aligned16(params + p->chain.w_off[1]) && aligned16(params + p->chain.w_off[2]) && aligned16(acts + p->chain.act_off[0]) &&
           aligned16(params + p->chain.b_off[0]) && (size_t)N * (p->n_classes | 1) <= 12288;
}

struct Pass {
    NetPlan* p; const float* params; int N; void* stream; char* base; float* acts; uint8_t* idx; void* scratch;
    Pass(NetPlan* plan, const float* prm, int n, void* ws, void* st)
        : p(plan), params(prm), N(n), stream(st), base(static_cast<char*>(ws)), acts(reinterpret_cast<float*>(base + plan->off_acts)),
          idx(reinterpret_cast<uint8_t*>(base + plan->off_idx)), scratch(base + plan->off_scratch) {}
    hipStream_t s() const { return as_stream(stream); }
    float* image(const WeightImage& im) const { return reinterpret_cast<float*>(base + p->off_wino + im.off); }
};

static int plan_conv_u(Conv kind, int mode, const float* in, const float* U, const float* bias, const float* mask_src, float* out,
                       uint8_t* pool_idx, int unpool, int N, int Cin, int Cout, int H, int W, int relu, hipStream_t s) {
    return kind == Conv::Bs3 ? clhip_internal_bs_conv_u(mode, in, U, bias, mask_src, out, pool_idx, unpool, N, Cin, Cout, H, W, relu, s)
                             : clhip_internal_wino_conv_u(mode, in, U, bias, mask_src, out, pool_idx, unpool, N, Cin, Cout, H, W, relu, s);
}

static int launch_conv_fwd(const Pass& c, const LayerPlan& L, const float* in, float* out, uint8_t* pool_idx, int relu) {
    const float* w = c.params + L.w_off; const float* b = c.params + L.b_off;
    switch (L.fwd) {
    case Conv::Wino: case Conv::Bs3:
        return plan_conv_u(L.fwd, 0, in, c.image(L.img_f), b, nullptr, out, pool_idx, 0, c.N, L.cin, L.cout, L.h, L.w, relu, c.s());
    case Conv::Direct3:
        return pool_idx ? clhip_conv3x3_relu_pool_fwd(in, w, b, out, pool_idx, c.N, L.cin, L.cout, L.h, L.w, c.stream)
                        : clhip_conv3x3_fwd(in, w, b, out, c.N, L.cin, L.cout, L.h, L.w, relu, c.stream);
    case Conv::Bs5:
        return clhip_internal_bs5_conv_u(0, in, c.image(L.img_f), b, nullptr, out, c.N, L.cin, L.cout, L.h, L.w, relu, c.s());
    case Conv::S2d:
        return clhip_conv2d_s2d_fwd(in, w, b, out, c.N, L.cin, L.h, L.w, L.cout, L.ks, L.st, L.pd, relu, c.base + c.p->off_s2d + L.s2d_off,
                                    L.s2d_bytes, c.stream);
    default:
        return clhip_conv2d_fwd(in, w, b, out, c.N, L.cin, L.h, L.w, L.cout, L.ks, L.ks, L.st, L.pd, relu, c.stream);
    }
}

static int launch_conv_bwd_data(const Pass& c, const LayerPlan& L, const float* dy, uint8_t* unpool_idx, const float* xmask, float* dx) {
    const float* w = c.params + L.w_off;
    switch (L.bwd) {
    case Conv::Wino: case Conv::Bs3:
        return plan_conv_u(L.bwd, 1, dy, c.image(L.img_d), nullptr, xmask, dx, unpool_idx, unpool_idx ? 1 : 0, c.N, L.cout, L.cin, L.h, L.w, 0,
                           c.s());
    case Conv::Direct3:
        return unpool_idx ? clhip_conv3x3_bwd_data_unpool(dy, unpool_idx, w, xmask, dx, c.N, L.cin, L.cout, L.h, L.w, c.stream)
                          : clhip_conv3x3_bwd_data(dy, w, xmask, dx, c.N, L.cin, L.cout, L.h, L.w, c.stream);
    case Conv::Bs5:
        return clhip_internal_bs5_conv_u(1, dy, c.image(L.img_d), nullptr, xmask, dx, c.N, L.cout, L.cin, L.h, L.w, 0, c.s());
    default:
        return clhip_conv2d_bwd_data(dy, w, xmask, dx, c.N, L.cin, L.h, L.w, L.cout, L.ks, L.ks, L.st, L.pd, c.stream);
    }
}

static int launch_wgrad(const Pass& c, float* grads, const LayerPlan& L, const float* xin, const float* dy, const uint8_t* unpool_idx, void* st,
                        bool defer, clhip_wgrad_job* slot, bool* job) {
    NetPlan* p = c.p;
    float* dw = grads + L.w_off; float* db = grads + L.b_off;
    void* slabs = c.base + p->off_wg + L.wg_off;
    int r;
    auto declined = [&]() { return r == CLHIP_ENOTSUP || r == CLHIP_ENOSPC; };
    auto slab_kernel = [&](auto partial) {
        r = partial(xin, dy, unpool_idx, dw, db, c.N, L.cin, L.cout, L.h, L.w, slabs, L.wg_bytes, as_stream(st), slot);
        if (r == 0) *job = true;
        return !declined();
    };
    const bool region = defer && (unpool_idx || L.wg_bytes);
    if (region && (L.wg & WG_BS) && slab_kernel(clhip_internal_bs_wgrad_partial)) return r;
    if (region && (L.wg & WG_WINO) && slab_kernel(clhip_internal_wino_wgrad_partial)) return r;
    if (defer && (L.wg & WG_3X3)) {
        *job = true;
        return clhip_internal_conv3x3_wgrad_partial(xin, dy, unpool_idx, dw, db, c.N, L.cin, L.cout, L.h, L.w, slabs, L.wg_bytes, st, slot);
    }
    if (unpool_idx)
        return clhip_conv3x3_bwd_weight_unpool(xin, dy, unpool_idx, dw, db, c.N, L.cin, L.cout, L.h, L.w, c.scratch, p->scratch_bytes, st);
    if (L.wg & WG_BS5) {
        r = clhip_internal_bs5_wgrad(xin, dy, dw, db, c.N, L.cin, L.cout, L.h, L.w, c.scratch, p->scratch_bytes, as_stream(st));
        if (!declined()) return r;
    }
    if (L.wg & WG_S2D) {
        const bool fresh = p->s2d_fresh_n == c.N;
        p->s2d_fresh_n = 0;
        return clhip_conv2d_s2d_bwd_weight(fresh ? nullptr : xin, dy, dw, db, c.N, L.cin, L.h, L.w, L.cout, L.ks, L.st, L.pd,
                                           c.base + p->off_s2d + L.s2d_off, L.s2d_bytes, st);
    }
    return (L.wg & WG_3X3) ? clhip_conv3x3_bwd_weight(xin, dy, dw, db, c.N, L.cin, L.cout, L.h, L.w, c.scratch, p->scratch_bytes, st)
                           : clhip_conv2d_bwd_weight(xin, dy, dw, db, c.N, L.cin, L.h, L.w, L.cout, L.ks, L.ks, L.st, L.pd, c.scratch,
                                                     p->scratch_bytes, st);
}

static void wino_collect(const Pass& c, bool fwd, bool bwd, std::vector<clhip_wino_wt>& jobs, std::vector<clhip_wino_wt>& bsjobs) {
    jobs.reserve(2 * c.p->layers.size());
    bsjobs.reserve(2 * c.p->layers.size());
    for (const LayerPlan& L : c.p->layers) {
        auto add = [&](const WeightImage& im, int ko, int ci, int mode) {
            const float* w = c.params + L.w_off;
            switch (im.kind) {
            case Img::WinoU: jobs.push_back(clhip_wino_wt{w, c.image(im), ko, ci, mode, 0}); break;
            case Img::Bs3: bsjobs.push_back(clhip_wino_wt{w, c.image(im), ko, ci, mode, 0}); break;
            case Img::Bs5: bsjobs.push_back(clhip_wino_wt{w, c.image(im), ko, ci, mode, 5}); break;
            case Img::None: break;
            }
        };
        if (fwd) add(L.img_f, L.cout, L.cin, 0);
        if (bwd) add(L.img_d, L.cin, L.cout, 1);
    }
}

static int wino_prepare(const Pass& c, bool fwd, bool bwd) {
    std::vector<clhip_wino_wt> jobs, bsjobs;
    wino_collect(c, fwd, bwd, jobs, bsjobs);
    return clhip_internal_weight_images(jobs.data(), (int)jobs.size(), bsjobs.data(), (int)bsjobs.size(), c.s());
}

static int net_forward_impl(void* handle, const float* params, const float* x, int N, void* ws, float* logits_out,
                            void* stream, int tail, int* slabs_live = nullptr, bool prep_bwd = false) {
    NetPlan* p = static_cast<NetPlan*>(handle);
    if (!p || !params || !x || !ws || N <= 0 || N > p->max_batch) return CLHIP_EINVAL;
    const Pass c(p, params, N, ws, stream);
    float* acts = c.acts;
    std::vector<clhip_wino_wt> edge_jobs, edge_bsjobs;
    bool edge = false;
    if (p->wino_bytes) {
        const LayerPlan& L0 = p->layers[0];
        edge = p->edge_grids && L0.fused_pool && L0.fwd == Conv::Direct3 && !L0.drop && L0.cin == 3;
// ... 14 lines not shown
            ~ProbeEnd() { if (on) { (void)hipEventRecord(p->probe_ev[2 * (p->probe_count % PROBE_RING) + 1], s); ++p->probe_count; } }
        } probe_end{p, probed, c.s()};
        if (L.drop && L.has_drop_buf) {
            float* dropped = acts + L.drop_off;
            rc = drop_copy(cur, dropped, L.drop, L.drop_stride, L.in_elems, N, c.s());
            if (rc) return rc;
            cur = dropped;
        } else if (L.drop) {
            rc = drop_scale(const_cast<float*>(cur), L.drop, L.drop_stride, L.in_elems, N, c.s());
            if (rc) return rc;
        }
        if (L.type == 0) {
            float* pl = acts + L.pool_off;
            uint8_t* pidx = c.idx + L.idx_off;
            if (li == 0 && edge) {
                rc = clhip_internal_c3w64_pool_weight_images(cur, params + L.w_off, params + L.b_off, pl, pidx, N, L.cin, L.cout,
                                                             L.h, L.w, edge_jobs.data(), (int)edge_jobs.size(), edge_bsjobs.data(),
                                                             (int)edge_bsjobs.size(), p->edge_grids == 2, c.s());
                if (rc == 0) { ++p->edge_count; cur = pl; continue; }
                if (rc != CLHIP_ENOTSUP) return rc;
                rc = clhip_internal_weight_images(edge_jobs.data(), (int)edge_jobs.size(), edge_bsjobs.data(), (int)edge_bsjobs.size(), c.s());
                if (rc) return rc;
            }
            float* zc = L.bn ? acts + L.z_off : L.fused_pool ? pl : y;
            rc = launch_conv_fwd(c, L, cur, zc, L.fused_pool ? pidx : nullptr, L.bn ? 0 : L.relu);
            if (rc) return rc;
            if (L.fwd == Conv::S2d) p->s2d_fresh_n = N;
            if (L.bn) {
                float* st = acts + L.stat_off;
                rc = clhip_bn_fwd(zc, params + L.bn_w_off, params + L.bn_b_off, L.rmean, L.rvar, y, st, st + L.cout, N, L.cout,
                                  L.oh * L.ow, p->training, L.bn_momentum, L.bn_eps, L.relu, c.scratch, p->scratch_bytes, stream);
                if (rc) return rc;
            }
            cur = L.fused_pool ? pl : y;
            if (L.pool && !L.fused_pool) {
                rc = L.pool22 ? clhip_maxpool2_fwd(y, pl, pidx, N * L.cout, L.oh, L.ow, stream)
                              : clhip_maxpool_fwd(y, pl, pidx, N * L.cout, L.oh, L.ow, L.pk, L.ps, stream);
                if (rc) return rc;
                cur = pl;
            }
        } else {
            if (tail && (int)li == p->fc_first) {
                rc = clhip_internal_fc_fwd_partial(cur, params + L.w_off, N, L.cin, L.cout, c.scratch, p->scratch_bytes, &live, c.s());
                if (rc) return rc;
            }
            if (!live) {
                rc = clhip_fc_fwd(cur, params + L.w_off, params + L.b_off, y, N, L.cin, L.cout, L.relu, c.scratch, p->scratch_bytes, stream);
                if (rc) return rc;
            }
            cur = y;
        }
    }
    if (slabs_live) *slabs_live = live;
    if (tail == 1) return 0;
    if (tail == 2) {
        rc = clhip_internal_fc_tail(&p->chain, params, acts, N, nullptr, 0, 0, 0, nullptr, nullptr, nullptr, nullptr,
                                    c.base + p->off_rows, p->tail_counter, 0, 0, static_cast<const float*>(c.scratch), live, c.s());
        if (rc) return rc;
        cur = acts + p->layers.back().act_off;
    }
    if (logits_out) {
        hipError_t e = hipMemcpyAsync(logits_out, cur, (size_t)N * p->n_classes * sizeof(float), hipMemcpyDeviceToDevice, c.s());
        if (e != hipSuccess) return (int)e;
    }
    return 0;
}

struct BackwardPass {
    const Pass c;
    NetPlan* const p;
    float* const grads; const float* const dlogits;
    float* const g[2]; float* const fcdz;
    const hipStream_t main_s;
    const bool ov;
    const bool ov_small;
    const bool defer;
    const float* gin;
    int gin_buf = -1;
    int flip = 0, taken = -1;
    hipEvent_t last_side = nullptr;
    hipEvent_t pending[2] = {nullptr, nullptr};
    clhip_wgrad_job jobs[CLHIP_WGRAD_JOBS_MAX];
    int n_jobs = 0;

    BackwardPass(NetPlan* plan, const float* params, float* grads_, int N, void* ws, const float* dl, void* stream)
        : c(plan, params, N, ws, stream), p(plan), grads(grads_), dlogits(dl),
          g{reinterpret_cast<float*>(c.base + plan->off_g0), reinterpret_cast<float*>(c.base + plan->off_g1)},
          fcdz(reinterpret_cast<float*>(c.base + plan->off_fcdz)), main_s(as_stream(stream)), ov(plan->overlap && plan->overlap_mode == 1),
          ov_small(plan->overlap && plan->overlap_mode == 2), defer(plan->n_wg > 0 && !ov), gin(dl) {}

    bool side_ok(int layer) const {
        const LayerPlan& Ls = p->layers[layer];
        return ov || (ov_small && Ls.type == 0 && (Ls.wg & WG_3X3) && Ls.h * Ls.w <= 256);
    }
    bool pair_ok(const LayerPlan& L, int layer) const {
        return defer && L.bwd == Conv::Wino && (L.wg & WG_WINO) && !(L.wg & WG_BS) && L.wg_bytes && !L.drop && !L.extra_grad && !side_ok(layer);
    }
    float* take() {
        const int bi = flip;
        flip ^= 1;
        if (pending[bi]) { (void)hipStreamWaitEvent(main_s, pending[bi], 0); pending[bi] = nullptr; }
        taken = bi;
        return g[bi];
    }
    template <class F> int on_side(int layer, int dy_buf, F&& launch) {
        if (!side_ok(layer)) return launch(c.stream);
        hipError_t e = hipEventRecord(p->ev_dy[layer], main_s);
        if (e == hipSuccess) e = hipStreamWaitEvent(p->side, p->ev_dy[layer], 0);
        if (e != hipSuccess) return (int)e;
        const int r = launch((void*)p->side);
        if (r) return r;
        e = hipEventRecord(p->ev_wg[layer], p->side);
        if (e != hipSuccess) return (int)e;
        last_side = p->ev_wg[layer];
        if (dy_buf >= 0) pending[dy_buf] = p->ev_wg[layer];
        return 0;
    }
    int finish_input_grad(const LayerPlan& L, float* gout) {
        if (L.drop) {
            const int rc = drop_scale(gout, L.drop, L.drop_stride, L.in_elems, c.N, main_s);
            if (rc) return rc;
        }
        return L.extra_grad ? add_inplace(gout, L.extra_grad, L.in_elems * (size_t)c.N, main_s) : 0;
    }
    int fc_layer(int i, const float* xin);
    int conv_layer(int i, const float* xin, const float* xmask);
};

int BackwardPass::fc_layer(int i, const float* xin) {
    const LayerPlan& L = p->layers[i];
    const int N = c.N;
    int rc;
    if (!p->fc_fused) {
        rc = clhip_fc_bwd_weight(xin, gin, grads + L.w_off, grads + L.b_off, N, L.cin, L.cout, c.scratch, p->scratch_bytes, c.stream);
        if (rc) return rc;
    }
    bool combo = false;
    clhip_fc_chain ch;
    if (p->fc_fused && i == p->fc_first) {
        ch = p->chain;
        for (int l = 1; l < ch.n; ++l) {
            const LayerPlan& Ll = p->layers[p->fc_first + l];
            if (Ll.drop && Ll.has_drop_buf) ch.act_off[l - 1] = Ll.drop_off;
        }
    }
    if (i > 0) {
        float* gout;
        if (p->fc_fused && i > p->fc_first) { gout = fcdz + p->chain.dz_off[i - p->fc_first - 1]; gin_buf = -1; }
        else { gout = take(); gin_buf = taken; }
        clhip_gemm_args ga;
        const int gb = (p->fc_fused && i == p->fc_first && !p->no_combo)
                           ? clhip_internal_fc_bwd_data_args(gin, c.params + L.w_off, xin, gout, N, L.cin, L.cout, &ga) : 0;
        if (gb > 0) {
            rc = clhip_internal_fc_bwd_combo(&ga, gb, &ch, grads, xin, N, c.acts, dlogits, fcdz, main_s);
            combo = true;
        } else {
            rc = clhip_fc_bwd_data(gin, c.params + L.w_off, xin, gout, N, L.cin, L.cout, c.scratch, p->scratch_bytes, c.stream);
        }
        if (rc) return rc;
        gin = gout;
        rc = finish_input_grad(L, gout);
        if (rc) return rc;
    }
    if (p->fc_fused && i == p->fc_first && !combo) {
        rc = clhip_internal_fc_chain_wgrad(&ch, grads, xin, N, c.acts, dlogits, fcdz, main_s);
        if (rc) return rc;
    }
    return 0;
}

int BackwardPass::conv_layer(int i, const float* xin, const float* xmask) {
    const LayerPlan& L = p->layers[i];
    const int N = c.N;
    uint8_t* const pidx = c.idx + L.idx_off;
    const float* gy = gin; int gy_buf = gin_buf;
    bool wdone = false, ddone = false;
    float* gout_d = nullptr; int gout_d_buf = -1;
    int rc;
    auto probe_on = [&](int kind) { return i == p->probe_layer && p->probe_kind == kind && !p->probe_ev.empty(); };
    auto probe_stream = [&](int kind) { return (kind == 2 && side_ok(i)) ? p->side : main_s; };
    auto probe_begin = [&](int kind) { if (probe_on(kind)) (void)hipEventRecord(p->probe_ev[2 * (p->probe_count % PROBE_RING)], probe_stream(kind)); };
    auto probe_end = [&](int kind) {
        if (probe_on(kind)) { (void)hipEventRecord(p->probe_ev[2 * (p->probe_count % PROBE_RING) + 1], probe_stream(kind)); ++p->probe_count; }
    };
    auto one_grid = [&](const float* dy, uint8_t* idx_or_null) {
        gout_d = take(); gout_d_buf = taken;
        if (p->probe_kind) probe_begin(p->probe_kind);
        const int r = clhip_internal_wino_pair(dy, idx_or_null, c.image(L.img_d), xmask, gout_d, xin, grads + L.w_off, grads + L.b_off, N, L.cin,
                                               L.cout, L.h, L.w, c.base + p->off_wg + L.wg_off, L.wg_bytes, main_s, &jobs[n_jobs]);
        if (r == 0) { wdone = ddone = true; ++n_jobs; if (p->probe_kind) probe_end(p->probe_kind); }
        return r == CLHIP_ENOTSUP ? 0 : r;
    };
    auto wgrad = [&](const float* dy, uint8_t* idx_or_null, int dy_buf) {
        bool job = false;
        probe_begin(2);
        const int r = on_side(i, dy_buf, [&](void* st) { return launch_wgrad(c, grads, L, xin, dy, idx_or_null, st, defer, &jobs[n_jobs], &job); });
        if (r == 0) { wdone = true; probe_end(2); if (job) ++n_jobs; }
        return r;
    };
    if (L.vgg && L.pool22 && !L.bn && (L.wg & WG_3X3)) {
        if (pair_ok(L, i)) {
            rc = one_grid(gin, pidx);
            if (rc) return rc;
        }
        if (!wdone) {
            rc = wgrad(gin, pidx, gin_buf);
            if (rc && rc != CLHIP_ENOTSUP) return rc;
        }
        if (wdone && !ddone && i > 0 && !L.drop && !L.extra_grad) {
            if (!gout_d) { gout_d = take(); gout_d_buf = taken; }
            probe_begin(1);
            rc = launch_conv_bwd_data(c, L, gin, pidx, xmask, gout_d);
            if (rc == 0) { ddone = true; probe_end(1); }
            else if (rc != CLHIP_ENOTSUP) return rc;
        }
    }
    if (L.pool && !(wdone && (i == 0 || ddone))) {
        float* gout = gout_d;
        if (gout) taken = gout_d_buf; else gout = take();
        rc = L.pool22 ? clhip_maxpool2_bwd(gin, pidx, gout, N * L.cout, L.oh, L.ow, c.stream)
                      : clhip_maxpool_bwd(gin, pidx, gout, N * L.cout, L.oh, L.ow, L.pk, L.ps, c.stream);
        if (rc) return rc;
        gy = gout; gy_buf = taken;
        gout_d = nullptr;
    }
    if (L.bn) {
        const float* st = c.acts + L.stat_off;
        float* dzb = const_cast<float*>(gy);
        if (gy_buf < 0) return CLHIP_EINVAL;
        rc = clhip_bn_bwd(gy, c.acts + L.act_off, c.acts + L.z_off, c.params + L.bn_w_off, st, st + L.cout, dzb, grads + L.bn_w_off,
                          grads + L.bn_b_off, N, L.cout, L.oh * L.ow, p->training, L.relu, c.scratch, p->scratch_bytes, c.stream);
        if (rc) return rc;
    }
    if (!wdone && !L.pool && !gout_d && pair_ok(L, i)) {
        rc = one_grid(gy, nullptr);
        if (rc) return rc;
    }
    if (!wdone) {
        rc = wgrad(gy, nullptr, gy_buf);
        if (rc) return rc;
    }
    if (ddone) { gin = gout_d; gin_buf = gout_d_buf; }
    if (i == 0 || ddone) return 0;
    float* gout = gout_d;
    if (gout) taken = gout_d_buf; else gout = take();
    probe_begin(1);
    rc = launch_conv_bwd_data(c, L, gy, nullptr, xmask, gout);
    if (rc) return rc;
    probe_end(1);
    gin = gout; gin_buf = taken;
    return finish_input_grad(L, gout);
}

static int net_backward_impl(void* handle, const float* params, float* grads, const float* x, int N, void* ws,
                             const float* dlogits, void* stream, bool tail_done, bool wino_ready = false) {
    NetPlan* p = static_cast<NetPlan*>(handle);
    if (!p || !params || !grads || !x || !ws || !dlogits || N <= 0 || N > p->max_batch) return CLHIP_EINVAL;
    BackwardPass b(p, params, grads, N, ws, dlogits, stream);
    int rc;
    if (p->wino_bytes && !wino_ready) {
        rc = wino_prepare(b.c, false, true);
        if (rc) return rc;
    }
    for (int i = (int)p->layers.size() - 1; i >= 0; --i) {
        const LayerPlan& L = p->layers[i];
        const float* xin = x;
        bool masked = true;
        if (i > 0) {
            const LayerPlan& P = p->layers[i - 1];
            xin = b.c.acts + ((P.type == 0 && P.pool) ? P.pool_off : P.act_off);
            if (L.drop && L.has_drop_buf) xin = b.c.acts + L.drop_off;
            masked = !(L.type == 0 && !L.drop && P.fused_pool);
        }
        if (L.type == 1 && tail_done && i > p->fc_first) {
            b.gin = b.fcdz + p->chain.dz_off[i - p->fc_first - 1]; b.gin_buf = -1;
            continue;
        }
        rc = L.type == 1 ? b.fc_layer(i, xin) : b.conv_layer(i, xin, masked ? xin : nullptr);
        if (rc) return rc;
    }
    if (b.last_side) {
        hipError_t e = hipStreamWaitEvent(b.main_s, b.last_side, 0);
        if (e != hipSuccess) return (int)e;
    }
    return b.n_jobs ? clhip_internal_wgrad_reduce_multi(b.jobs, b.n_jobs, b.main_s) : 0;
}

}

extern "C" {

int clhip_net_create(const clhip_layer_desc* descs, int n_layers, int max_batch, int in_c, int in_h, int in_w,
                     void** out_handle) {
    if (!descs || n_layers <= 0 || max_batch <= 0 || !out_handle) return CLHIP_EINVAL;
    std::unique_ptr<NetPlan> p(new (std::nothrow) NetPlan());
    if (!p) return CLHIP_ENOSPC;
    p->max_batch = max_batch; p->in_c = in_c; p->in_h = in_h; p->in_w = in_w;
    p->in_elems = (size_t)in_c * in_h * in_w;
    const int rc = plan_geometry(*p, descs, n_layers);
    if (rc) return rc;
    for (int i = 0; i < n_layers; ++i)
        if (p->layers[i].type == 0) choose_paths(p->layers[i], descs[i], i, max_batch);
    layout_arena(*p);
    make_resources(*p);
    *out_handle = p.release();
    return 0;
}

int clhip_net_set_dropout(void* handle, int layer, const float* mask, long row_stride) {
    NetPlan* p = static_cast<NetPlan*>(handle);
    if (!p || layer <= 0 || layer >= (int)p->layers.size() || row_stride < 0) return CLHIP_EINVAL;
    p->layers[layer].drop = mask;
    p->layers[layer].drop_stride = row_stride;
    return 0;
}

int clhip_net_set_bn(void* handle, int layer, float* running_mean, float* running_var, float momentum, float eps) {
    NetPlan* p = static_cast<NetPlan*>(handle);
    if (!p || layer < 0 || layer >= (int)p->layers.size() || !p->layers[layer].bn || !(eps > 0.f)) return CLHIP_EINVAL;
    LayerPlan& L = p->layers[layer];
    L.rmean = running_mean; L.rvar = running_var; L.bn_momentum = momentum; L.bn_eps = eps;
    return 0;
}

int clhip_net_layer_input(void* handle, int layer, size_t* ws_float_off, size_t* in_elems) {
    NetPlan* p = static_cast<NetPlan*>(handle);
    if (!p || layer <= 0 || layer >= (int)p->layers.size() || !ws_float_off || !in_elems) return CLHIP_EINVAL;
    const LayerPlan& P = p->layers[layer - 1];
    *ws_float_off = p->off_acts / sizeof(float) + ((P.type == 0 && P.pool) ? P.pool_off : P.act_off);
    *in_elems = p->layers[layer].in_elems;
    return 0;
}

int clhip_net_layer_pool_idx(void* handle, int layer, size_t* ws_byte_off, size_t* elems) {
    NetPlan* p = static_cast<NetPlan*>(handle);
    if (!p || layer < 0 || layer >= (int)p->layers.size() || !ws_byte_off || !elems) return CLHIP_EINVAL;
    const LayerPlan& L = p->layers[layer];
    if (L.type != 0 || !L.pool) return CLHIP_EINVAL;
    *ws_byte_off = p->off_idx + L.idx_off;
    *elems = L.pool_elems;
    return 0;
}

int clhip_net_edge_grid_count(void* handle) {
    NetPlan* p = static_cast<NetPlan*>(handle);
    return p ? (int)(p->edge_count & 0x7fffffffu) : CLHIP_EINVAL;
}

int clhip_net_prepared_weights(void* handle, size_t* ws_byte_off, size_t* bytes) {
    NetPlan* p = static_cast<NetPlan*>(handle);
    if (!p || !ws_byte_off || !bytes) return CLHIP_EINVAL;
    *ws_byte_off = p->off_wino;
    *bytes = p->wino_bytes;
    return 0;
}

int clhip_net_layer_paths(void* handle, int layer) {
    NetPlan* p = static_cast<NetPlan*>(handle);
    if (!p || layer < 0 || layer >= (int)p->layers.size()) return CLHIP_EINVAL;
    const LayerPlan& L = p->layers[layer];
    if (L.type == 1) {
        bool tail = p->fc_tail && layer > p->fc_first;
        for (size_t i = p->fc_first + 1; tail && i < p->layers.size(); ++i)
            if (p->layers[i].drop || p->layers[i].extra_grad) tail = false;
        return (tail ? 64 : 0) | ((p->fc_fused && layer >= p->fc_first) ? 128 : 0);
    }
    auto dir = [](Conv k) { return (k == Conv::Wino || k == Conv::Bs3 ? 1 : 0) | (k == Conv::Bs3 || k == Conv::Bs5 ? 8 : 0); };
    const bool defer_capable = p->n_wg > 0 && !(p->overlap && p->overlap_mode == 1);
    return dir(L.fwd) | dir(L.bwd) << 1 | (((L.wg & WG_WINO) && defer_capable) ? 4 : 0) | (((L.wg & WG_BS) && defer_capable) ? 32 : 0);
}

int clhip_net_set_input_grad(void* handle, int layer, const float* extra) {
    NetPlan* p = static_cast<NetPlan*>(handle);
    if (!p || layer <= 0 || layer >= (int)p->layers.size()) return CLHIP_EINVAL;
    p->layers[layer].extra_grad = extra;
    return 0;
}

int clhip_net_probe(void* handle, int layer) {
    NetPlan* p = static_cast<NetPlan*>(handle);
    if (!p || layer >= (int)p->layers.size()) return CLHIP_EINVAL;
    if (layer >= 0 && p->probe_ev.empty()) {
        std::vector<hipEvent_t> made;
        made.reserve(2 * PROBE_RING);
        for (unsigned i = 0; i < 2 * PROBE_RING; ++i) {
            hipEvent_t e;
            if (hipEventCreate(&e) != hipSuccess) {
                for (hipEvent_t m : made) (void)hipEventDestroy(m);
                return CLHIP_ENOTSUP;
            }
            made.push_back(e);
        }
        p->probe_ev.swap(made);
    }
    p->probe_layer = layer;
    p->probe_kind = 0;
    p->probe_count = 0;
    return 0;
}

int clhip_net_probe_kind(void* handle, int layer, int kind) {
    if (kind < 0 || kind > 2) return CLHIP_EINVAL;
    const int rc = clhip_net_probe(handle, layer);
    if (rc == 0) static_cast<NetPlan*>(handle)->probe_kind = kind;
    return rc;
}

int clhip_net_probe_read(void* handle, float* avg_us, int* count) {
    NetPlan* p = static_cast<NetPlan*>(handle);
    if (!p || !avg_us || !count) return CLHIP_EINVAL;
    const unsigned n = p->probe_count < PROBE_RING ? p->probe_count : PROBE_RING;
    double sum = 0.0;
    for (unsigned i = 0; i < n; ++i) {
        const unsigned slot = (p->probe_count - 1 - i) % PROBE_RING;
        float ms = 0.f;
        hipError_t e = hipEventSynchronize(p->probe_ev[2 * slot + 1]);
        if (e == hipSuccess) e = hipEventElapsedTime(&ms, p->probe_ev[2 * slot], p->probe_ev[2 * slot + 1]);
        if (e != hipSuccess) return (int)e;
        sum += ms;
    }
    *avg_us = n ? (float)(sum / n * 1e3) : 0.f;
    *count = (int)n;
    p->probe_count = 0;
    return 0;
}

int clhip_net_set_training(void* handle, int training) {
    NetPlan* p = static_cast<NetPlan*>(handle);
    if (!p) return CLHIP_EINVAL;
    p->training = training ? 1 : 0;
    return 0;
// ... 87 lines not shown
```

### clsurvey_amd/net.py

```python
import ctypes as C
import weakref

import torch
import torch.nn as nn

from . import _lib
from ._lib import check, LayerDesc


def _pad4(n):
    return (n + 3) // 4 * 4


class ParamArena:
    _registry = weakref.WeakValueDictionary()

    @classmethod
    def find(cls, params):
        params = list(params)
        if not params:
            return None
        a = cls._registry.get(id(params[0]))
        if a is None or len(a.params) != len(params) or any(x is not y for x, y in zip(a.params, params)):
            return None
# ... 151 lines not shown
            d.relu, d.pool = int(relu), int(bool(pool))
            if isinstance(pool, tuple):
                d.pool_k, d.pool_s = int(pool[0]), int(pool[1])
            if kind == "conv":
                d.ksize, d.stride, d.pad = (int(v) for v in (sp[7] if len(sp) > 7 else (w.shape[2], 1, w.shape[2] // 2)))
            d.w_off = self.arena.slot(w)[0]
            d.b_off = self.arena.slot(b)[0]
        for li in self.drops:
            descs[li].has_drop = 1
        for li, bn in self.bns.items():
            descs[li].bn = 1
            descs[li].bn_w_off = self.arena.slot(bn.weight)[0]
            descs[li].bn_b_off = self.arena.slot(bn.bias)[0]
        self.max_batch = int(max_batch)
        self.in_shape = tuple(in_shape)
        h = C.c_void_p()
        L = _lib.lib()
        check(L.clhip_net_create(descs, len(specs), self.max_batch, *self.in_shape, C.byref(h)),
              "clhip_net_create")
        self._h = h
        self.n_classes = L.clhip_net_num_classes(h)
        self.ws = torch.empty(L.clhip_net_workspace_bytes(h), dtype=torch.uint8, device=self.device)
        self.loss = torch.zeros(1, dtype=torch.float32, device=self.device)
        for li, bn in self.bns.items():
            for name in ("running_mean", "running_var", "num_batches_tracked"):
                buf = getattr(bn, name)
                buf.data = buf.data.to(self.device).contiguous()
            check(L.clhip_net_set_bn(h, li, bn.running_mean.data_ptr(), bn.running_var.data_ptr(), float(bn.momentum), float(bn.eps)),
                  "clhip_net_set_bn")
        self._training = None
        self.in_elems = {}
        shp = self.in_shape
        if self.drops:
            with torch.no_grad():
                c, h, w = shp
                for li, sp in enumerate(specs):
                    self.in_elems[li] = c * h * w
                    if sp[0] == "conv":
                        ks, st, pd = sp[7] if len(sp) > 7 else (3, 1, 1)
                        c, h, w = sp[4], (h + 2 * pd - ks) // st + 1, (w + 2 * pd - ks) // st + 1
                        if sp[6]:
                            pk, ps = sp[6] if isinstance(sp[6], tuple) else (2, 2)
                            h, w = (h - pk) // ps + 1, (w - pk) // ps + 1
                    else:
                        c, h, w = sp[4], 1, 1
        self.auto_dropout = True
        self._masks = {}

    def set_dropout(self, layer, mask):
        if mask is None:
            self._masks.pop(layer, None)
            ptr, stride = None, 0
        else:
            if not mask.is_cuda or mask.dtype != torch.float32 or not mask.is_contiguous():
                raise RuntimeError("dropout masks are contiguous fp32 HIP tensors")
            if mask.shape[-1] != self.in_elems[layer] or (mask.dim() == 2 and mask.shape[0] < 1):
                raise RuntimeError("dropout mask shape %s does not fit layer %d" % (tuple(mask.shape), layer))
            self._masks[layer] = mask
            ptr, stride = mask.data_ptr(), (mask.shape[-1] if mask.dim() == 2 else 0)
        check(_lib.lib().clhip_net_set_dropout(self._h, int(layer), ptr, int(stride)), "clhip_net_set_dropout")

    def layer_input(self, layer, n):
        off, elems = C.c_size_t(), C.c_size_t()
        check(_lib.lib().clhip_net_layer_input(self._h, int(layer), C.byref(off), C.byref(elems)), "clhip_net_layer_input")
        lo = off.value * 4
        return self.ws[lo:lo + n * elems.value * 4].view(torch.float32).view(n, elems.value)

    def pool_idx(self, layer, n):
        off, elems = C.c_size_t(), C.c_size_t()
        check(_lib.lib().clhip_net_layer_pool_idx(self._h, int(layer), C.byref(off), C.byref(elems)), "clhip_net_layer_pool_idx")
        return self.ws[off.value:off.value + n * elems.value].view(n, elems.value)

    def prepared_weights(self):
        off, nbytes = C.c_size_t(), C.c_size_t()
        check(_lib.lib().clhip_net_prepared_weights(self._h, C.byref(off), C.byref(nbytes)), "clhip_net_prepared_weights")
        return self.ws[off.value:off.value + nbytes.value]

    def edge_grid_count(self):
        n = _lib.lib().clhip_net_edge_grid_count(self._h)
        if n < 0:
            raise RuntimeError("clhip_net_edge_grid_count")
        return n

    def layer_paths(self, layer):
        bits = _lib.lib().clhip_net_layer_paths(self._h, int(layer))
        if bits < 0:
            raise RuntimeError("clhip_net_layer_paths(%d)" % layer)
        return {"fwd": bool(bits & 1), "bwd_data": bool(bits & 2), "bwd_weight": bool(bits & 4),
                "bs_fwd": bool(bits & 8), "bs_bwd_data": bool(bits & 16), "bs_bwd_weight": bool(bits & 32),
                "fc_tail": bool(bits & 64), "fc_fused": bool(bits & 128)}

    def set_input_grad(self, layer, extra):
        if extra is not None and (not extra.is_cuda or extra.dtype != torch.float32 or not extra.is_contiguous()):
            raise RuntimeError("set_input_grad needs a contiguous fp32 HIP tensor")
        self._extra = extra
        check(_lib.lib().clhip_net_set_input_grad(self._h, int(layer), extra.data_ptr() if extra is not None else None),
              "clhip_net_set_input_grad")

    def _mode(self):
        if not self.bns:
            return
        training = bool(self.model.training)
        if training != self._training:
            check(_lib.lib().clhip_net_set_training(self._h, int(training)), "clhip_net_set_training")
            self._training = training
        if training:
            for bn in self.bns.values():
                bn.num_batches_tracked += 1

    def probe(self, layer, kind="fwd"):
        k = {"fwd": 0, "bwd_data": 1, "bwd_weight": 2}[kind]
        check(_lib.lib().clhip_net_probe_kind(self._h, -1 if layer is None else int(layer), k), "clhip_net_probe_kind")

    def probe_read(self):
        import ctypes as C
        us, n = C.c_float(0.0), C.c_int(0)
        check(_lib.lib().clhip_net_probe_read(self._h, C.byref(us), C.byref(n)), "clhip_net_probe_read")
        return float(us.value), int(n.value)

    def _auto_drop(self, n):
        if not self.drops or not self.auto_dropout:
            return
        for li, m in self.drops.items():
            if self.model.training and m.p > 0:
                keep = 1.0 - m.p
                mask = torch.empty((n, self.in_elems[li]), dtype=torch.float32, device=self.device).bernoulli_(keep).div_(keep)
                self.set_dropout(li, mask)
            elif li in self._masks:
                self.set_dropout(li, None)

    def __del__(self):
        try:
            if getattr(self, "_h", None):
                _lib.lib().clhip_net_destroy(self._h)
                self._h = None
        except Exception:
            pass

    def _check_x(self, x):
        if not x.is_cuda or x.dtype != torch.float32 or not x.is_contiguous():
            raise RuntimeError("NetEngine needs contiguous fp32 HIP tensors")
        if tuple(x.shape[1:]) != self.in_shape or x.shape[0] > self.max_batch:
            raise RuntimeError("NetEngine: bad input shape %s" % (tuple(x.shape),))

    def forward(self, x, params=None):
        self._check_x(x)
        self._mode()
        self._auto_drop(x.shape[0])
        logits = torch.empty((x.shape[0], self.n_classes), dtype=torch.float32, device=self.device)
        check(_lib.lib().clhip_net_forward(self._h, (params if params is not None else self.arena.theta).data_ptr(),
                                           x.data_ptr(), x.shape[0],
                                           self.ws.data_ptr(), logits.data_ptr(),
                                           torch.cuda.current_stream().cuda_stream), "clhip_net_forward")
        return logits

    def backward(self, x, dlogits):
        self._check_x(x)
        check(_lib.lib().clhip_net_backward(self._h, self.arena.theta.data_ptr(), self.arena.grad.data_ptr(), x.data_ptr(),
                                            x.shape[0], self.ws.data_ptr(), dlogits.data_ptr(),
                                            torch.cuda.current_stream().cuda_stream), "clhip_net_backward")

    def loss_step(self, x, y, kind="ce_mean", backward=True, stats=None, want_logits=False, params=None,
                  class_slice=None):
        self._check_x(x)
        self._mode()
        self._auto_drop(x.shape[0])
# ... 24 lines not shown
```

### include/clhip.h

```cpp
#ifndef CLHIP_H
#define CLHIP_H

#include <stddef.h>
#include <stdint.h>

#ifdef __cplusplus
extern "C" {
#endif

#if defined(__GNUC__) || defined(__clang__)
#pragma GCC visibility push(default)
#define CLHIP_VISIBILITY_PUSHED 1
#endif

#define CLHIP_EINVAL (-1)
#define CLHIP_ENOSPC (-2)
#define CLHIP_ENOTSUP (-3)

int clhip_sigmoid_fwd(const float* x, float* y, size_t n, void* stream);
int clhip_sigmoid_bwd(const float* dy, const float* y, float* dx, size_t n, void* stream);
int clhip_mse_mean(const float* a, const float* b, size_t n, float grad_scale, float* da, float* loss_out, void* stream);
int clhip_adadelta_step(float* theta, const float* grad, float* square_avg, float* acc_delta, size_t n, float lr, float rho,
                        float eps, float weight_decay, void* stream);

// ... 42 lines not shown
size_t clhip_conv2d_bwd_weight_ws(int N, int C, int H, int W, int K, int R, int S, int stride, int pad);
int clhip_conv2d_fwd(const float* x, const float* w, const float* b, float* y, int N, int C, int H, int W, int K, int R, int S,
                     int stride, int pad, int relu, void* stream);
int clhip_conv2d_bwd_data(const float* dy, const float* w, const float* relu_src, float* dx, int N, int C, int H, int W, int K,
                          int R, int S, int stride, int pad, void* stream);
int clhip_conv2d_bwd_weight(const float* x, const float* dy, float* dw, float* db, int N, int C, int H, int W, int K, int R,
                            int S, int stride, int pad, void* ws, size_t ws_bytes, void* stream);

size_t clhip_conv3x3_bs_bwd_weight_ws(int N, int C, int K, int H, int W);
int clhip_conv3x3_bs_bwd_weight(const float* x, const float* dy, const uint8_t* idx_u8_or_null, float* dw, float* db, int N, int C, int K,
                                int H, int W, void* ws, size_t ws_bytes, void* stream);

size_t clhip_conv5x5_bs_bwd_weight_ws(int N, int C, int K, int H, int W);
int clhip_conv5x5_bs_bwd_weight(const float* x, const float* dy, float* dw, float* db, int N, int C, int K, int H, int W, void* ws,
                                size_t ws_bytes, void* stream);

size_t clhip_conv2d_s2d_ws(int N, int C, int H, int W, int K, int R, int stride, int pad);
int clhip_conv2d_s2d_fwd(const float* x, const float* w, const float* b, float* y, int N, int C, int H, int W, int K, int R, int stride,
                         int pad, int relu, void* ws, size_t ws_bytes, void* stream);
int clhip_conv2d_s2d_bwd_weight(const float* x_or_null, const float* dy, float* dw, float* db, int N, int C, int H, int W, int K, int R,
                                int stride, int pad, void* ws, size_t ws_bytes, void* stream);

size_t clhip_fc_ws(int M, int I, int O);
int clhip_fc_fwd(const float* x, const float* w, const float* b, float* y,
                 int M, int I, int O, int relu, void* ws, size_t ws_bytes, void* stream);
int clhip_fc_bwd_data(const float* dy, const float* w, const float* relu_src, float* dx,
                      int M, int I, int O, void* ws, size_t ws_bytes, void* stream);
int clhip_fc_bwd_weight(const float* x, const float* dy, float* dw, float* db,
                        int M, int I, int O, void* ws, size_t ws_bytes, void* stream);
int clhip_relu_bwd(const float* dy, const float* y, float* dx, size_t n, void* stream);

int clhip_softmax_ce(const float* logits, const int64_t* labels_i64, int N, int C, int reduction,
                     float* dlogits, float* loss_out, double* stats, void* stream);
int clhip_softmax_ce_slice(const float* logits, const int64_t* labels_i64, int N, int ld, int col_off, int ncols,
                           int reduction, float* dlogits, float* loss_out, double* stats, void* stream);
int clhip_mse_zero_sum(const float* logits, size_t n, float* dlogits, float* loss_out, void* stream);

int clhip_lwf_loss(const float* logits, const int64_t* labels_i64, const float* teacher, const int* head_sizes, int n_heads,
                   int N, int ld, int ld_teacher, float T, float reg_lambda, int distill, float* dlogits, float* loss_out2,
                   double* stats, void* stream);

int clhip_reg_sgd_step(float* theta, const float* grad, const float* omega, const float* init_val,
                       float* buf, size_t n, float reg_lambda, float lr, float momentum, float wd,
                       int first, void* stream);
int clhip_fisher_accum(float* omega, const float* grad, size_t n, float data_len, void* stream);
int clhip_mas_accum(float* omega, const float* grad, size_t n, float prev_size, float curr_size,
                    void* stream);
int clhip_si_step(float* theta, const float* grad, const float* omega, const float* init_val,
                  float* w, float* buf, size_t n, float reg_lambda, float lr, float momentum,
                  float wd, int first, void* stream);
int clhip_si_consolidate(float* omega, float* w, const float* theta, float* init_val, size_t n,
                         float slack, void* stream);

int clhip_imm_merge(const float* const* thetas, const float* const* precisions, const float* sum_precision,
                    int n_models, size_t n, float* out, void* stream);

int clhip_packnet_finetune_mask(uint8_t* mask_u8, size_t n, int cur, void* stream);
size_t clhip_packnet_kth_ws(void);
int clhip_packnet_kth_abs(const float* w, const uint8_t* mask_u8, size_t n, int cur, size_t k,
                          float* out_cutoff, void* ws, size_t ws_bytes, void* stream);
int clhip_packnet_prune(float* w, uint8_t* mask_u8, size_t n, int cur, const float* cutoff_dev, void* stream);
int clhip_mask_grad_zero(float* grad, const uint8_t* mask_u8, size_t n, int cur, void* stream);
int clhip_mask_weight_zero(float* w, const uint8_t* mask_u8, size_t n, int mode, int idx, void* stream);
int clhip_packnet_sgd_step(float* theta, float* grad, float* buf, const uint8_t* mask_u8, size_t n, int cur,
                           float lr, float momentum, float wd, int first, void* stream);

size_t clhip_conv3x3_wino_ws(int C, int K);
int clhip_conv3x3_wino_fwd(const float* x, const float* w, const float* b, float* y, uint8_t* idx_u8_or_null, int N, int C, int K,
                           int H, int W, int relu, void* ws, size_t ws_bytes, void* stream);
int clhip_conv3x3_wino_bwd_data(const float* dy, const uint8_t* idx_u8_or_null, const float* w, const float* relu_src, float* dx,
                                int N, int C, int K, int H, int W, void* ws, size_t ws_bytes, void* stream);
size_t clhip_conv3x3_wino_bwd_weight_ws(int N, int C, int K, int H, int W);
int clhip_conv3x3_wino_bwd_weight(const float* x, const float* dy, const uint8_t* idx_u8_or_null, float* dw, float* db, int N, int C,
                                  int K, int H, int W, void* ws, size_t ws_bytes, void* stream);
size_t clhip_conv3x3_wino_bwd_ws(int N, int C, int K, int H, int W);
int clhip_conv3x3_wino_bwd(const float* x, const float* dy, const uint8_t* idx_u8_or_null, const float* w, const float* relu_src,
                           float* dx, float* dw, float* db, int N, int C, int K, int H, int W, void* ws, size_t ws_bytes, void* stream);

size_t clhip_conv3x3_bs_ws(int C, int K);
int clhip_conv3x3_bs_fwd(const float* x, const float* w, const float* b, float* y, uint8_t* idx_u8_or_null, int N, int C, int K,
                         int H, int W, int relu, void* ws, size_t ws_bytes, void* stream);
int clhip_conv3x3_bs_bwd_data(const float* dy, const uint8_t* idx_u8_or_null, const float* w, const float* relu_src, float* dx,
                              int N, int C, int K, int H, int W, void* ws, size_t ws_bytes, void* stream);
size_t clhip_conv5x5_bs_ws(int C, int K);
int clhip_conv5x5_bs_fwd(const float* x, const float* w, const float* b, float* y, int N, int C, int K, int H, int W, int relu,
                         void* ws, size_t ws_bytes, void* stream);
int clhip_conv5x5_bs_bwd_data(const float* dy, const float* w, const float* relu_src, float* dx, int N, int C, int K, int H, int W,
                              void* ws, size_t ws_bytes, void* stream);

int clhip_hat_gate(const float* emb_row, int n, float s, float* gate, void* stream);
int clhip_hat_scale_weight(const float* w, const float* gate_in, float* out, size_t K, size_t C, size_t R, void* stream);
int clhip_hat_weight_grad(const float* g_wprime, const float* w, const float* gate_in, float* dw, float* dgate_in,
                          int K, int C, int R, void* stream);
int clhip_hat_emb_grad(const float* dgate, const float* gate, const float* mask_pre, int n, float s,
                       float lamb_over_count, float* demb, void* stream);
int clhip_hat_reg_sums(const float* gate, const float* mask_pre, int n, double* sums2, void* stream);
int clhip_hat_backmask(const float* a_post, const float* a_pre, float* out, size_t K, size_t C, size_t R, void* stream);
size_t clhip_hat_sgd_ws(void);
int clhip_hat_sgd_step(float* theta, float* grad, float* buf, const float* mask_back, size_t n, float lr,
                       float momentum, float wd, int is_emb, int finetune, float s, float smax, float thres_cosh,
                       float clipgrad, int first, void* ws, size_t ws_bytes, void* stream);
int clhip_clamp(float* x, size_t n, float lo, float hi, void* stream);

typedef struct { float* theta; float* grad; float* buf; const float* mask_back; size_t n; int is_emb; int reserved; } clhip_hat_param;
typedef struct { const float* emb_row; float* gate; const float* mask_pre; int n; int reserved; } clhip_hat_gate_job;
typedef struct { const float* w; const float* gate_in; float* out; size_t K, C, R; } clhip_hat_layer;
typedef struct { float* g; const float* w; const float* gate_in; float* dgate_in; int K, C, R, reserved; } clhip_hat_wgrad_job;
typedef struct { const float* dgate; const float* gate; const float* mask_pre; float* demb; int n, rows, t, reserved; } clhip_hat_emb_job;
size_t clhip_hat_sgd_multi_ws(int n_params);
int clhip_hat_sgd_step_multi(const clhip_hat_param* params, int n_params, float lr, float momentum, float wd, int finetune,
                             float s, float smax, float thres_cosh, float clipgrad, float thres_emb, int first, void* ws,
                             size_t ws_bytes, void* stream);
int clhip_hat_gates_multi(const clhip_hat_gate_job* jobs, int n_jobs, float s, double* sums2, void* stream);
int clhip_hat_scale_weights_multi(const clhip_hat_layer* layers, int n_layers, void* stream);
int clhip_hat_weight_grads_multi(const clhip_hat_wgrad_job* jobs, int n_jobs, void* stream);
int clhip_hat_emb_grads_multi(const clhip_hat_emb_job* jobs, int n_jobs, float s, float lamb, float count, const double* sums2,
                              void* stream);

#define CLHIP_PATHNET_MAX_N 8
#define CLHIP_PATHNET_MAX_LAYERS 24
typedef struct {
    long w_off, b_off;
    long pw_off, pb_off;
    long mod_stride;
    int c_out, c_in, R;
    int n_out, n_in;
    int Kp, Cp;
    int M;
    int path[CLHIP_PATHNET_MAX_N];
    unsigned long long trainable;
} clhip_pathnet_layer;
size_t clhip_pathnet_ws(const clhip_pathnet_layer* layers, int n_layers);
int clhip_pathnet_pack_multi(const clhip_pathnet_layer* layers, int n_layers, const float* mod_theta, size_t mod_numel,
                             float* packed_theta, size_t packed_numel, void* stream);
int clhip_pathnet_fold_grads_multi(const clhip_pathnet_layer* layers, int n_layers, const float* packed_grad, size_t packed_numel,
                                   float* mod_grad, size_t mod_numel, void* ws, size_t ws_bytes, void* stream);
int clhip_pathnet_sgd_step(const clhip_pathnet_layer* layers, int n_layers, float* mod_theta, float* mod_grad, float* mod_buf,
                           size_t mod_numel, float lr, float momentum, float wd, float clipgrad, int first, const void* ws,
                           size_t ws_bytes, void* stream);

typedef struct {
    int type;
    int cin, cout;
    int relu, pool;
    long w_off, b_off;
    int ksize, stride, pad;
    int pool_k, pool_s;
    int bn;
    long bn_w_off, bn_b_off;
    int has_drop;
} clhip_layer_desc;

int clhip_net_create(const clhip_layer_desc* layers, int n_layers, int max_batch, int in_c, int in_h,
                     int in_w, void** out_handle);
int clhip_net_set_dropout(void* handle, int layer, const float* mask, long row_stride);
int clhip_net_set_bn(void* handle, int layer, float* running_mean, float* running_var, float momentum, float eps);
int clhip_net_set_training(void* handle, int training);
int clhip_net_probe(void* handle, int layer);
int clhip_net_probe_kind(void* handle, int layer, int kind);
int clhip_net_probe_read(void* handle, float* avg_us, int* count);
int clhip_net_layer_pool_idx(void* handle, int layer, size_t* ws_byte_off, size_t* elems_per_sample);
int clhip_net_prepared_weights(void* handle, size_t* ws_byte_off, size_t* bytes);
int clhip_net_edge_grid_count(void* handle);
int clhip_net_layer_paths(void* handle, int layer);

int clhip_net_layer_input(void* handle, int layer, size_t* ws_float_off, size_t* in_elems);
int clhip_net_set_input_grad(void* handle, int layer, const float* extra);
void clhip_net_destroy(void* handle);
size_t clhip_net_workspace_bytes(void* handle);
int clhip_net_num_classes(void* handle);
int clhip_net_forward(void* handle, const float* params, const float* x, int N, void* ws,
                      float* logits_out, void* stream);
int clhip_net_backward(void* handle, const float* params, float* grads, const float* x, int N, void* ws,
                       const float* dlogits, void* stream);
int clhip_net_loss_step(void* handle, const float* params, float* grads, const float* x,
                        const int64_t* labels_i64, int N, int loss_kind, void* ws, float* loss_out,
                        double* stats, float* logits_out, void* stream);

int clhip_net_loss_step_slice(void* handle, const float* params, float* grads, const float* x,
                              const int64_t* labels_i64, int N, int loss_kind, int col_off, int ncols, void* ws,
                              float* loss_out, double* stats, float* logits_out, void* stream);

int clhip_axpy(float* y, const float* x, size_t n, float alpha, int assign, void* stream);
size_t clhip_gem_gram_ws(int m);
int clhip_gem_gram(const float* G, size_t ld, const int* row_idx_host, int m, size_t n, double* out_f64, void* ws,
                   size_t ws_bytes, void* stream);
int clhip_gem_project(const float* G, size_t ld, const int* row_idx_host, const float* v_host, int m, const float* g,
                      float* out, size_t n, void* stream);
int clhip_gem_qp(const double* gram_f64, int m, double margin, double eps, double* v_out_f64, int* info_i32, void* stream);
int clhip_gem_project_dev(const float* G, size_t ld, const int* row_idx_host, const double* v_dev_f64, const int* info_dev,
                          int m, const float* g, float* out, size_t n, void* stream);
#define CLHIP_GEM_WIDE_MAX 64
size_t clhip_gem_gram_wide_ws(int m);
int clhip_gem_gram_wide(const float* G, size_t ld, const int* row_idx_host, int m, size_t n, double* out_f64, void* ws,
                        size_t ws_bytes, void* stream);
size_t clhip_gem_qp_wide_ws(int m);
int clhip_gem_qp_wide(const double* gram_f64, int m, double margin, double eps, double* v_out_f64, int* info_i32, void* ws,
                      size_t ws_bytes, void* stream);
int clhip_gem_project_wide(const float* G, size_t ld, const int* row_idx_host, const float* v_host, int m, const float* g,
                           float* out, size_t n, void* stream);
int clhip_gem_project_dev_wide(const float* G, size_t ld, const int* row_idx_host, const double* v_dev_f64, const int* info_dev,
                               int m, const float* g, float* out, size_t n, void* stream);

#define CLHIP_LOSS_MAX_ROWS 1024
#define CLHIP_LOSS_MAX_SEGS 256
typedef struct clhip_loss_segment { int row_begin; int row_end; int col_off; int ncols; float scale; int kind; } clhip_loss_segment;
int clhip_rehearsal_assemble(const float* x, const int64_t* labels_i64, int B, size_t row_elems, float* store_x,
                             int64_t* store_labels, long store_rows, long ring_row0, int ring_rows, const int* gather_rows,
                             int E, float* x_mix, int64_t* labels_mix, void* stream);
int clhip_rehearsal_assemble_crop_flip(const float* x, const int64_t* labels_i64, int B, int C, int Hs, int Ws, int th, int tw,
                                       const float* src_frames, long src_rows, const int64_t* src_idx, float* store_frames,
                                       int64_t* store_labels, long store_rows, long ring_row0, int ring_rows,
                                       const int* gather_rows, const int* gather_params, int E, float* x_mix, int64_t* labels_mix,
                                       void* stream);
int clhip_rehearsal_assemble_resized_crop_flip(const float* x, const int64_t* labels_i64, int B, int C, int Hs, int Ws, int th,
                                               int tw, const float* src_frames, long src_rows, const int64_t* src_idx,
                                               float* store_frames, int64_t* store_labels, long store_rows, long ring_row0,
                                               int ring_rows, const int* gather_rows, const int* gather_params, int E, float* x_mix,
                                               int64_t* labels_mix, void* stream);
int clhip_loss_segments(const float* logits, const int64_t* labels_i64, const float* targets, int ld_t, int N, int ld,
                        const clhip_loss_segment* segs, int n_segs, float T, float* dlogits, float* loss_out, double* stats,
                        void* stream);
int clhip_net_loss_step_loss_segments(void* handle, const float* params, float* grads, const float* x,
                                      const int64_t* labels_i64, const float* targets, int ld_t, int N,
                                      const clhip_loss_segment* segs, int n_segs, float T, void* ws, float* loss_out,
                                      double* stats, float* logits_out, void* stream);

#define CLHIP_MAX_TASKS 64
typedef struct clhip_task_src { const float* x; const int64_t* labels; int64_t cum_rows; int64_t label_shift; } clhip_task_src;
int clhip_gather_tasks(const clhip_task_src* tasks_dev, int T, size_t row_elems, const int64_t* idx, int B, float* x_out,
                       int64_t* labels_out, void* stream);
int clhip_slice_argmax_count(const float* logits, int N, int ld, const int* cols, int K, const int64_t* labels_i64,
                             int64_t* correct, int64_t* total, int64_t* out_of_range, void* stream);

int clhip_gather_tasks_crop_flip(const clhip_task_src* tasks_dev, int T, int C, int Hs, int Ws, int th, int tw, const int64_t* idx,
                                 const int* params, int B, float* x_out, int64_t* labels_out, void* stream);

#define CLHIP_RESIZE_MAX_RATIO 8
int clhip_gather_tasks_resized_crop_flip(const clhip_task_src* tasks_dev, int T, int C, int Hs, int Ws, int th, int tw,
                                         const int64_t* idx, const int* params, int B, float* x_out, int64_t* labels_out,
                                         void* stream);

typedef struct clhip_task_src_u8 { const uint8_t* x; const int64_t* labels; int64_t cum_rows; int64_t label_shift; } clhip_task_src_u8;
int clhip_gather_tasks_u8(const clhip_task_src_u8* tasks_dev, int T, int C, size_t plane_elems, const float* lut,
                          const int64_t* idx, int B, float* x_out, int64_t* labels_out, void* stream);
int clhip_gather_tasks_crop_flip_u8(const clhip_task_src_u8* tasks_dev, int T, int C, int Hs, int Ws, int th, int tw, const float* lut,
// ... 56 lines not shown
```

Baseline: 303,900 images/s.

## Fuse deferred weight-gradient split reductions into a conv backward-data launch as rider blocks

Adds a bs_conv_riders kernel that appends extra 'rider' blocks to a 3x3 backward-data conv grid. These blocks run the deferred weight-gradient slab reductions that previously needed their own launch. The backward pass picks a host layer, passes the pending reduce jobs to that layer's bwd-data call, and clears the jobs once they have run. The goal is to save a kernel launch and fill idle or tail slots in the conv grid. The cost is mixing workloads in one kernel, which can lower occupancy through the combined launch bounds and adds placement logic (place modes 1-3).

```diff
diff --git a/clsurvey_amd/_lib.py b/clsurvey_amd/_lib.py
--- a/clsurvey_amd/_lib.py
+++ b/clsurvey_amd/_lib.py
@@ -39,6 +39,10 @@
 
 class IcarlClass(C.Structure):
     _fields_ = [("row_begin", _i), ("row_end", _i), ("k", _i), ("out_off", _i)]
+
+
+class ReduceJob(C.Structure):
+    _fields_ = [("slabs", _p), ("dw", _p), ("db", _p), ("K", _i), ("C", _i), ("splits", _i), ("taps", _i)]
 
 
 class LayerDesc(C.Structure):
@@ -68,6 +72,7 @@
     "clhip_conv3x3_bs_ws": (_z, [_i, _i]),
     "clhip_conv3x3_bs_fwd": (_i, [_p, _p, _p, _p, _p, _i, _i, _i, _i, _i, _i, _p, _z, _p]),
     "clhip_conv3x3_bs_bwd_data": (_i, [_p, _p, _p, _p, _p, _i, _i, _i, _i, _i, _p, _z, _p]),
+    "clhip_conv3x3_bs_bwd_data_riders": (_i, [_p, _p, _p, _p, _p, _i, _i, _i, _i, _i, _p, _z, C.POINTER(ReduceJob), _i, _i, _i, _p]),
     "clhip_conv3x3_wino_bwd_weight_ws": (_z, [_i, _i, _i, _i, _i]),
     "clhip_conv3x3_wino_bwd_weight": (_i, [_p, _p, _p, _p, _p, _i, _i, _i, _i, _i, _p, _z, _p]),
     "clhip_conv3x3_wino_bwd_ws": (_z, [_i, _i, _i, _i, _i]),
@@ -151,6 +156,7 @@
     "clhip_net_layer_pool_idx": (_i, [_p, _i, _p, _p]),
     "clhip_net_prepared_weights": (_i, [_p, _p, _p]),
     "clhip_net_edge_grid_count": (_i, [_p]),
+    "clhip_net_reduce_rider_count": (_i, [_p]),
     "clhip_net_layer_paths": (_i, [_p, _i]),
     "clhip_net_probe_kind": (_i, [_p, _i, _i]),
     "clhip_net_set_input_grad": (_i, [_p, _i, _p]),
diff --git a/clsurvey_amd/csrc/bsconv.hip b/clsurvey_amd/csrc/bsconv.hip
--- a/clsurvey_amd/csrc/bsconv.hip
+++ b/clsurvey_amd/csrc/bsconv.hip
@@ -1,5 +1,6 @@
 #include "common.hpp"
 #include "bs_weight.hpp"
+#include "wgrad_reduce.hpp"
 #include <cstdlib>
 
 #ifndef BS_ABL
@@ -404,6 +405,51 @@
     }
 }
 
+template <class GA, class GB>
+constexpr bool bs_same_geo() { return GA::RW == GB::RW && GA::RH == GB::RH && GA::NI == GB::NI && GA::WM == GB::WM; }
+
+template <class GA, class GB, bool UNPOOL>
+__global__ __launch_bounds__(256, (bs_blocks_per_cu<GA, UNPOOL>() < bs_blocks_per_cu<GB, UNPOOL>() ? bs_blocks_per_cu<GA, UNPOOL>()
+                                                                                                  : bs_blocks_per_cu<GB, UNPOOL>()))
+void bs_conv_riders_kernel(const float* __restrict__ in, const clhip_u32x4* __restrict__ wimg, const float* __restrict__ mask_src,
+                           float* __restrict__ out, uint8_t* __restrict__ pool_idx, int N, int Cin, int Cout, int H, int W, int blocks_a,
+                           int NA, int tiles_xa, int tiles_ya, int npb_a, int tiles_xb, int tiles_yb, int npb_b, int place, int riders,
+                           int stride, RedJobs jobs) {
+    constexpr int LB = 2 * (GA::BUF_BYTES > GB::BUF_BYTES ? GA::BUF_BYTES : GB::BUF_BYTES);
+    static_assert(LB >= (int)(RED_J * RED_EL * sizeof(double)) && RED_THREADS == 256, "a rider is one reduction block inside the host's block");
+    __shared__ __attribute__((aligned(16))) unsigned char lds[LB];
+    int b = (int)blockIdx.x, r = -1;
+    if (place == 1) {
+        if (b < riders) r = b; else b -= riders;
+    } else if (place == 3) {
+        const int g = b >> 3, rg = riders >> 3, q = g / stride;
+        if (g - q * stride == stride - 1 && q < rg) r = q * 8 + (b & 7);
+        else { const int before = (g + 1) / stride; b -= 8 * (before < rg ? before : rg); }
+    } else {
+        const int conv_blocks = (int)gridDim.x - riders;
+        if (b >= conv_blocks) r = b - conv_blocks;
+    }
+    if (r >= 0) {
+        double (*partial)[RED_EL] = reinterpret_cast<double (*)[RED_EL]>(lds);
+        const unsigned units = jobs.first[jobs.n];
+        for (unsigned u = (unsigned)r; u < units; u += (unsigned)riders) {
+            wgrad_reduce_unit<RED_EL, RED_J>(jobs, u, partial);
+            __syncthreads();
+        }
+        return;
+    }
+    if (bs_same_geo<GA, GB>() || b < blocks_a) {
+        bs_conv_body<GA, 1, UNPOOL>(lds, b, in, wimg, nullptr, mask_src, out, pool_idx, NA, Cin, Cout, H, W, 0, tiles_xa, tiles_ya, npb_a);
+    } else if constexpr (!bs_same_geo<GA, GB>()) {
+        const size_t in_img = (size_t)Cin * (UNPOOL ? (size_t)(H >> 1) * (W >> 1) : (size_t)H * W);
+        const size_t out_img = (size_t)Cout * H * W;
+        uint8_t* idx_b = pool_idx ? pool_idx + (size_t)NA * in_img : nullptr;
+        bs_conv_body<GB, 1, UNPOOL>(lds, b - blocks_a, in + (size_t)NA * in_img, wimg, nullptr,
+                                    mask_src ? mask_src + (size_t)NA * out_img : nullptr, out + (size_t)NA * out_img, idx_b, N - NA, Cin, Cout,
+                                    H, W, 0, tiles_xb, tiles_yb, npb_b);
+    }
+}
+
 
 static int bs_env_int(const char* name, int dflt) {
     const char* e = getenv(name);
@@ -424,28 +470,40 @@
     return 0;
 }
 
-template <int MODE, bool UNPOOL>
-int bs_launch_mixed32(const float* in, const clhip_u32x4* wimg, const float* bias, const float* mask_src, float* out, uint8_t* pool_idx,
-                      int N, int Cin, int Cout, int H, int W, int relu, hipStream_t s, bool* taken) {
-    using GA = BsGeo<32, 4, 1, 2, 2, 1>;
-    using GB = BsGeo<32, 2, 1, 2, 1, 1>;
-    *taken = false;
+using BsGA32 = BsGeo<32, 4, 1, 2, 2, 1>;
+using BsGB32 = BsGeo<32, 2, 1, 2, 1, 1>;
+struct BsMixed { int blocks_a, NA, txa, tya, npb_a, txb, tyb, npb_b; long long blocks; };
+
+template <bool UNPOOL>
+bool bs_mixed32_plan(int N, int Cout, int H, int W, BsMixed& m) {
+    using GA = BsGA32;
+    using GB = BsGB32;
     static const int on = bs_env_int("CLHIP_BS_MIXED", 1);
-    if (!on) return 0;
+    if (!on) return false;
     const int kts = (Cout + BS_BN - 1) / BS_BN;
     const long long per_img_a = (long long)((W + GA::RW - 1) / GA::RW) * ((H + GA::RH - 1) / GA::RH);
     const long long slots = 256LL * bs_blocks_per_cu<GA, UNPOOL>();
     const long long total = per_img_a * N * kts, rounds = total / slots, rem = total - rounds * slots;
-    if (rounds < 1 || rem == 0 || 2 * rem > slots) return 0;
+    if (rounds < 1 || rem == 0 || 2 * rem > slots) return false;
     const long long na = rounds * slots / (per_img_a * kts);
-    if (na < 1 || na >= N || na % 8) return 0;
-    const int NA = (int)na;
-    const int txa = (W + GA::RW - 1) / GA::RW, tya = (H + GA::RH - 1) / GA::RH, txb = (W + GB::RW - 1) / GB::RW, tyb = (H + GB::RH - 1) / GB::RH;
-    const long long npb_a = (long long)txa * tya * NA, npb_b = (long long)txb * tyb * (N - NA);
+    if (na < 1 || na >= N || na % 8) return false;
+    m.NA = (int)na;
+    m.txa = (W + GA::RW - 1) / GA::RW; m.tya = (H + GA::RH - 1) / GA::RH; m.txb = (W + GB::RW - 1) / GB::RW; m.tyb = (H + GB::RH - 1) / GB::RH;
+    const long long npb_a = (long long)m.txa * m.tya * m.NA, npb_b = (long long)m.txb * m.tyb * (N - m.NA);
     const long long blocks_a = (npb_a + 7) / 8 * 8 * kts, blocks_b = (npb_b + 7) / 8 * 8 * kts;
-    if (blocks_a + blocks_b > 0x7fffffffLL) return 0;
-    hipLaunchKernelGGL((bs_conv_mixed_kernel<GA, GB, MODE, UNPOOL>), dim3((unsigned)(blocks_a + blocks_b)), dim3(256), 0, s, in, wimg, bias,
-                       mask_src, out, pool_idx, N, Cin, Cout, H, W, relu, (int)blocks_a, NA, txa, tya, (int)npb_a, txb, tyb, (int)npb_b);
+    if (blocks_a + blocks_b > 0x7fffffffLL) return false;
+    m.npb_a = (int)npb_a; m.npb_b = (int)npb_b; m.blocks_a = (int)blocks_a; m.blocks = blocks_a + blocks_b;
+    return true;
+}
+
+template <int MODE, bool UNPOOL>
+int bs_launch_mixed32(const float* in, const clhip_u32x4* wimg, const float* bias, const float* mask_src, float* out, uint8_t* pool_idx,
+                      int N, int Cin, int Cout, int H, int W, int relu, hipStream_t s, bool* taken) {
+    *taken = false;
+    BsMixed m;
+    if (!bs_mixed32_plan<UNPOOL>(N, Cout, H, W, m)) return 0;
+    hipLaunchKernelGGL((bs_conv_mixed_kernel<BsGA32, BsGB32, MODE, UNPOOL>), dim3((unsigned)m.blocks), dim3(256), 0, s, in, wimg, bias,
+                       mask_src, out, pool_idx, N, Cin, Cout, H, W, relu, m.blocks_a, m.NA, m.txa, m.tya, m.npb_a, m.txb, m.tyb, m.npb_b);
     CLHIP_LAUNCH_CHECK();
     *taken = true;
     return 0;
@@ -464,6 +522,46 @@
     if (W > 8) BS_GO(16, 8, 1, 2, 2, 1);
     BS_GO(8, 8, 2, 2, 2, 1);
 #undef BS_GO
+}
+
+template <class GA, class GB, bool UNPOOL>
+int bs_launch_riders_geo(const float* in, const clhip_u32x4* wimg, const float* mask_src, float* out, uint8_t* pool_idx, int N, int Cin,
+                         int Cout, int H, int W, const BsMixed& m, const RedJobs& jobs, int place, int riders, hipStream_t s) {
+    const long long total = m.blocks + riders;
+    if (m.blocks <= 0 || total > 0x7fffffffLL) return CLHIP_ENOTSUP;
+    const int stride = (int)((total / 8) / (riders / 8));
+    if (place == 3 && stride < 2) place = 2;
+    hipLaunchKernelGGL((bs_conv_riders_kernel<GA, GB, UNPOOL>), dim3((unsigned)total), dim3(256), 0, s, in, wimg, mask_src, out, pool_idx, N,
+                       Cin, Cout, H, W, m.blocks_a, m.NA, m.txa, m.tya, m.npb_a, m.txb, m.tyb, m.npb_b, place, riders, stride, jobs);
+    CLHIP_LAUNCH_CHECK();
+    return 0;
+}
+
+template <class G>
+BsMixed bs_one_geo(int N, int Cout, int H, int W) {
+    BsMixed m{};
+    m.txa = (W + G::RW - 1) / G::RW; m.tya = (H + G::RH - 1) / G::RH; m.NA = N;
+    const long long npb = (long long)m.txa * m.tya * ((N + G::NI - 1) / G::NI);
+    const long long blocks = (npb + 7) / 8 * 8 * ((Cout + BS_BN - 1) / BS_BN);
+    m.blocks = (npb > 0x7fffffffLL || blocks > 0x7fffffffLL) ? 0 : blocks;
+    m.npb_a = (int)npb; m.blocks_a = (int)m.blocks;
+    return m;
+}
+
+template <bool UNPOOL>
+int bs_launch_riders(const float* in, const clhip_u32x4* wimg, const float* mask_src, float* out, uint8_t* pool_idx, int N, int Cin,
+                     int Cout, int H, int W, const RedJobs& jobs, int place, int riders, hipStream_t s) {
+#define BS_RIDE(GA_, GB_, M_) return bs_launch_riders_geo<GA_, GB_, UNPOOL>(in, wimg, mask_src, out, pool_idx, N, Cin, Cout, H, W, M_, jobs, place, riders, s)
+    if (W > 16 && !((H | W) & 1)) {
+        BsMixed m;
+        if (bs_mixed32_plan<UNPOOL>(N, Cout, H, W, m)) BS_RIDE(BsGA32, BsGB32, m);
+    }
+    using G16 = BsGeo<16, 8, 1, 2, 2, 1>;
+    using G8 = BsGeo<8, 8, 2, 2, 2, 1>;
+    if (W > 16) BS_RIDE(BsGA32, BsGA32, bs_one_geo<BsGA32>(N, Cout, H, W));
+    if (W > 8) BS_RIDE(G16, G16, bs_one_geo<G16>(N, Cout, H, W));
+    BS_RIDE(G8, G8, bs_one_geo<G8>(N, Cout, H, W));
+#undef BS_RIDE
 }
 
 template <int MODE>
@@ -536,6 +634,29 @@
     return bs_launch<1, false>(in, img, nullptr, mask_src, out, nullptr, N, Cin, Cout, H, W, 0, s);
 }
 
+int clhip_internal_bs_conv_u_riders(const float* in, const void* wimg, const float* mask_src, float* out, uint8_t* pool_idx, int unpool,
+                                    int N, int Cin, int Cout, int H, int W, const clhip_wgrad_job* jobs, int n_jobs, int place,
+                                    int riders, hipStream_t s) {
+    if (!in || !wimg || !out || N <= 0 || !clhip_internal_bs_ok(Cin, Cout, H, W) || !clhip_internal_bs_index_ok(Cin, Cout, H, W, 3)) return CLHIP_EINVAL;
+    if (((H | W) & 1) && (pool_idx || unpool)) return CLHIP_ENOTSUP;
+    if (!jobs || n_jobs < 1 || n_jobs > CLHIP_WGRAD_JOBS_MAX || place < 1 || place > 3 || riders < 8 || riders % 8 || riders > (1 << 20))
+        return CLHIP_ENOTSUP;
+    unsigned long long units = 0;
+    for (int i = 0; i < n_jobs; ++i) {
+        const clhip_wgrad_job& j = jobs[i];
+        if (!j.part || !j.dw || j.K <= 0 || j.C <= 0 || j.splits <= 0 || (j.taps != 0 && j.taps != 9 && j.taps != 25)) return CLHIP_ENOTSUP;
+        units += ((unsigned long long)(j.taps ? j.taps : 9) * j.K * j.C + j.K + RED_EL - 1) / RED_EL;
+    }
+    if (units > 0x7fffffffULL) return CLHIP_ENOTSUP;
+    const int useful = (int)((units + 7) / 8 * 8);
+    if (riders > useful) riders = useful;
+    RedJobs r;
+    wgrad_reduce_fill(r, jobs, n_jobs);
+    const clhip_u32x4* img = static_cast<const clhip_u32x4*>(wimg);
+    if (unpool) return bs_launch_riders<true>(in, img, mask_src, out, pool_idx, N, Cin, Cout, H, W, r, place, riders, s);
+    return bs_launch_riders<false>(in, img, mask_src, out, nullptr, N, Cin, Cout, H, W, r, place, riders, s);
+}
+
 int clhip_internal_bs5_conv_u(int mode, const float* in, const void* wimg, const float* bias, const float* mask_src, float* out, int N,
                               int Cin, int Cout, int H, int W, int relu, hipStream_t s) {
     if (!in || !wimg || !out || N <= 0 || !clhip_internal_bs_ok(Cin, Cout, H, W) || W <= 8 || !clhip_internal_bs_index_ok(Cin, Cout, H, W, 5))
@@ -604,4 +725,26 @@
                                     N, K, C, H, W, 0, as_stream(stream));
 }
 
-}
+int clhip_conv3x3_bs_bwd_data_riders(const float* dy, const uint8_t* idx_u8_or_null, const float* w, const float* relu_src, float* dx, int N,
+                                     int C, int K, int H, int W, void* ws, size_t ws_bytes, const clhip_reduce_job* jobs, int n_jobs,
+                                     int place, int riders, void* stream) {
+    if (N <= 0 || !clhip_internal_bs_ok(K, C, H, W)) return CLHIP_ENOTSUP;
+    if (!dy || !w || !dx || !ws || ws_bytes < clhip_internal_bs_ws(K, C)) return CLHIP_EINVAL;
+    if (!clhip_internal_bs_index_ok(K, C, H, W, 3)) return CLHIP_EINVAL;
+    if (((H | W) & 1) && idx_u8_or_null) return CLHIP_ENOTSUP;
+    if (!jobs || n_jobs < 1 || n_jobs > CLHIP_WGRAD_JOBS_MAX || place < 1 || place > 3 || riders < 8 || riders % 8 || riders > (1 << 20))
+        return CLHIP_ENOTSUP;
+    clhip_wgrad_job q[CLHIP_WGRAD_JOBS_MAX];
+    for (int i = 0; i < n_jobs; ++i) {
+        const clhip_reduce_job& j = jobs[i];
+        if (!j.slabs || !j.dw || j.K <= 0 || j.C <= 0 || j.splits <= 0 || (j.taps != 9 && j.taps != 25)) return CLHIP_EINVAL;
+        q[i] = clhip_wgrad_job{j.slabs, j.dw, j.db, j.K, j.C, j.splits, j.taps};
+    }
+    const clhip_wino_wt job{w, static_cast<float*>(ws), C, K, 1, 0};
+    const int rc = clhip_internal_bs_weights(&job, 1, as_stream(stream));
+    if (rc) return rc;
+    return clhip_internal_bs_conv_u_riders(dy, ws, relu_src, dx, const_cast<uint8_t*>(idx_u8_or_null), idx_u8_or_null != nullptr, N, K, C, H,
+                                           W, q, n_jobs, place, riders, as_stream(stream));
+}
+
+}
diff --git a/clsurvey_amd/csrc/common.hpp b/clsurvey_amd/csrc/common.hpp
--- a/clsurvey_amd/csrc/common.hpp
+++ b/clsurvey_amd/csrc/common.hpp
@@ -166,6 +166,9 @@
 int clhip_internal_bs_weights(const clhip_wino_wt* jobs, int n, hipStream_t s);
 int clhip_internal_bs_conv_u(int mode, const float* in, const void* wimg, const float* bias, const float* mask_src, float* out,
                              uint8_t* pool_idx, int unpool, int N, int Cin, int Cout, int H, int W, int relu, hipStream_t s);
+int clhip_internal_bs_conv_u_riders(const float* in, const void* wimg, const float* mask_src, float* out, uint8_t* pool_idx, int unpool,
+                                    int N, int Cin, int Cout, int H, int W, const clhip_wgrad_job* jobs, int n_jobs, int place,
+                                    int riders, hipStream_t s);
 bool clhip_internal_bs5_wgrad_ok(int N, int C, int K, int H, int W);
 size_t clhip_internal_bs5_wgrad_ws(int N, int C, int K, int H, int W);
 int clhip_internal_bs5_wgrad(const float* x, const float* dy, float* dw, float* db, int N, int C, int K, int H, int W, void* ws,
diff --git a/clsurvey_amd/csrc/conv3x3_wgrad.hip b/clsurvey_amd/csrc/conv3x3_wgrad.hip
--- a/clsurvey_amd/csrc/conv3x3_wgrad.hip
+++ b/clsurvey_amd/csrc/conv3x3_wgrad.hip
@@ -1,5 +1,6 @@
 #include <cstdlib>
 #include "common.hpp"
+#include "wgrad_reduce.hpp"
 
 namespace {
 
@@ -692,49 +693,6 @@
     }
 }
 
-constexpr int RED_EL = 64, RED_J = 16, RED_V = 4;
-constexpr int RED_THREADS = RED_EL / RED_V * RED_J;
-
-template <int EL, int J>
-__device__ __forceinline__ void wgrad_reduce_block(const float* __restrict__ part, float* __restrict__ dw, float* __restrict__ db,
-                                                   int K, int C, int splits, size_t e0, double (*partial)[EL], int T = 9) {
-    const size_t kc = (size_t)K * C, nw = (size_t)T * kc, total = nw + K;
-    const int v = threadIdx.x % (EL / RED_V), j = threadIdx.x / (EL / RED_V);
-    const size_t e = e0 + (size_t)v * RED_V;
-    const int q = (splits + J - 1) / J;
-    const int s0 = j * q, s1 = min(splits, s0 + q);
-    double s[RED_V] = {0.0, 0.0, 0.0, 0.0};
-    if ((total & 3) == 0 && (reinterpret_cast<uintptr_t>(part) & 15u) == 0 && e + RED_V <= total) {
-#pragma unroll 4
-        for (int sp = s0; sp < s1; ++sp) {
-            const float4 t = *reinterpret_cast<const float4*>(part + (size_t)sp * total + e);
-            s[0] += (double)t.x; s[1] += (double)t.y; s[2] += (double)t.z; s[3] += (double)t.w;
-        }
-    } else {
-        for (int sp = s0; sp < s1; ++sp)
-#pragma unroll
-            for (int t = 0; t < RED_V; ++t)
-                if (e + t < total) s[t] += (double)part[(size_t)sp * total + e + t];
-    }
-#pragma unroll
-    for (int t = 0; t < RED_V; ++t) partial[j][v * RED_V + t] = s[t];
-    __syncthreads();
-    if (threadIdx.x < EL) {
-        const int el = threadIdx.x;
-        const size_t ee = e0 + el;
-        if (ee < total) {
-            double t = 0.0;
-#pragma unroll
-            for (int jj = 0; jj < J; ++jj) t += partial[jj][el];
-            if (ee < nw) {
-                const size_t rs = ee / kc, rem = ee - rs * kc;
-                dw[rem * T + rs] = (float)t;
-            } else if (db) {
-                db[ee - nw] = (float)t;
-            }
-        }
-    }
-}
 
 template <int EL, int J>
 __global__ __launch_bounds__(RED_THREADS) void wgrad_reduce_kernel(const float* __restrict__ part, float* __restrict__ dw,
@@ -743,19 +701,10 @@
     wgrad_reduce_block<EL, J>(part, dw, db, K, C, splits, (size_t)blockIdx.x * EL, partial);
 }
 
-struct RedJobs {
-    clhip_wgrad_job job[CLHIP_WGRAD_JOBS_MAX];
-    unsigned first[CLHIP_WGRAD_JOBS_MAX + 1];
-    int n;
-};
-
 template <int EL, int JL>
 __global__ __launch_bounds__(RED_THREADS) void wgrad_reduce_multi_kernel(RedJobs jobs) {
     __shared__ double partial[JL][EL];
-    int ji = 0;
-    while (ji + 1 < jobs.n && blockIdx.x >= jobs.first[ji + 1]) ++ji;
-    const clhip_wgrad_job J = jobs.job[ji];
-    wgrad_reduce_block<EL, JL>(J.part, J.dw, J.db, J.K, J.C, J.splits, (size_t)(blockIdx.x - jobs.first[ji]) * EL, partial, J.taps ? J.taps : 9);
+    wgrad_reduce_unit<EL, JL>(jobs, blockIdx.x, partial);
 }
 
 struct WPlan {
@@ -910,14 +859,7 @@
     if (n <= 0) return 0;
     if (!jobs || n > CLHIP_WGRAD_JOBS_MAX) return CLHIP_EINVAL;
     RedJobs r;
-    r.n = n;
-    r.first[0] = 0;
-    for (int i = 0; i < n; ++i) {
-        r.job[i] = jobs[i];
-        const size_t total = (size_t)(jobs[i].taps ? jobs[i].taps : 9) * jobs[i].K * jobs[i].C + jobs[i].K;
-        r.first[i + 1] = r.first[i] + (unsigned)((total + RED_EL - 1) / RED_EL);
-    }
-    for (int i = n; i < CLHIP_WGRAD_JOBS_MAX; ++i) { r.job[i] = clhip_wgrad_job{nullptr, nullptr, nullptr, 0, 0, 0, 0}; r.first[i + 1] = r.first[n]; }
+    wgrad_reduce_fill(r, jobs, n);
     hipLaunchKernelGGL((wgrad_reduce_multi_kernel<RED_EL, RED_J>), dim3(r.first[n]), dim3(RED_THREADS), 0, s, r);
     CLHIP_LAUNCH_CHECK();
     return 0;
diff --git a/clsurvey_amd/csrc/engine.hip b/clsurvey_amd/csrc/engine.hip
--- a/clsurvey_amd/csrc/engine.hip
+++ b/clsurvey_amd/csrc/engine.hip
@@ -65,6 +65,9 @@
 #ifndef CLHIP_EDGE_GRIDS_DEFAULT
 #define CLHIP_EDGE_GRIDS_DEFAULT 1
 #endif
+#ifndef CLHIP_REDUCE_RIDERS_DEFAULT
+#define CLHIP_REDUCE_RIDERS_DEFAULT 1
+#endif
 #ifndef CLHIP_OVERLAP_DEFAULT
 #define CLHIP_OVERLAP_DEFAULT 0
 #endif
@@ -78,6 +81,16 @@
 int edge_grids_mode() {
     const char* e = std::getenv("CLHIP_EDGE_GRIDS");
     return (e && e[0] >= '0' && e[0] <= '2' && !e[1]) ? e[0] - '0' : CLHIP_EDGE_GRIDS_DEFAULT;
+}
+
+int reduce_riders_mode() {
+    const char* e = std::getenv("CLHIP_REDUCE_RIDERS");
+    return (e && e[0] >= '0' && e[0] <= '3' && !e[1]) ? e[0] - '0' : CLHIP_REDUCE_RIDERS_DEFAULT;
+}
+int reduce_rider_blocks() {
+    const char* e = std::getenv("CLHIP_REDUCE_RIDER_BLOCKS");
+    const int v = e && e[0] ? std::atoi(e) : 0;
+    return (v > 0 && v % 256 == 0 && v <= 16384) ? v : 256;
 }
 
 struct NetPlan {
@@ -106,6 +119,8 @@
     size_t off_rows;
     int edge_grids;
     unsigned edge_count;
+    int reduce_riders, rider_blocks, rider_host = -1;
+    unsigned rider_count;
     bool overlap;
     int overlap_mode;
     hipStream_t side;
@@ -342,6 +357,10 @@
         } else { (void)hipGetLastError(); p.side = nullptr; }
     }
     p.edge_grids = edge_grids_mode();
+    p.reduce_riders = reduce_riders_mode();
+    p.rider_blocks = reduce_rider_blocks();
+    for (size_t i = n_layers; i-- > 1;)
+        if (p.layers[i].type == 0 && p.layers[i].bwd == Conv::Bs3) p.rider_host = (int)i;
     const bool tail = fc_tail_enabled();
     p.no_combo = !tail;
     if (p.fc_fused && tail && clhip_internal_fc_tail_ok(&p.chain) && p.max_batch <= 1024) {
@@ -397,10 +416,17 @@
     }
 }
 
-static int launch_conv_bwd_data(const Pass& c, const LayerPlan& L, const float* dy, uint8_t* unpool_idx, const float* xmask, float* dx) {
+static int launch_conv_bwd_data(const Pass& c, const LayerPlan& L, const float* dy, uint8_t* unpool_idx, const float* xmask, float* dx,
+                                const clhip_wgrad_job* ride = nullptr, int n_ride = 0, bool* rode = nullptr) {
     const float* w = c.params + L.w_off;
     switch (L.bwd) {
     case Conv::Wino: case Conv::Bs3:
+        if (ride && L.bwd == Conv::Bs3) {
+            const int r = clhip_internal_bs_conv_u_riders(dy, c.image(L.img_d), xmask, dx, unpool_idx, unpool_idx ? 1 : 0, c.N, L.cout, L.cin,
+                                                          L.h, L.w, ride, n_ride, c.p->reduce_riders, c.p->rider_blocks, c.s());
+            if (r == 0) *rode = true;
+            if (r != CLHIP_ENOTSUP) return r;
+        }
         return plan_conv_u(L.bwd, 1, dy, c.image(L.img_d), nullptr, xmask, dx, unpool_idx, unpool_idx ? 1 : 0, c.N, L.cout, L.cin, L.h, L.w, 0,
                            c.s());
     case Conv::Direct3:
@@ -581,6 +607,7 @@
     hipEvent_t pending[2] = {nullptr, nullptr};
     clhip_wgrad_job jobs[CLHIP_WGRAD_JOBS_MAX];
     int n_jobs = 0;
+    bool side_jobs = false;
 
     BackwardPass(NetPlan* plan, const float* params, float* grads_, int N, void* ws, const float* dl, void* stream)
         : c(plan, params, N, ws, stream), p(plan), grads(grads_), dlogits(dl),
@@ -694,7 +721,14 @@
         bool job = false;
         probe_begin(2);
         const int r = on_side(i, dy_buf, [&](void* st) { return launch_wgrad(c, grads, L, xin, dy, idx_or_null, st, defer, &jobs[n_jobs], &job); });
-        if (r == 0) { wdone = true; probe_end(2); if (job) ++n_jobs; }
+        if (r == 0) { wdone = true; probe_end(2); if (job) { ++n_jobs; side_jobs = side_jobs || side_ok(i); } }
+        return r;
+    };
+    auto bwd_data = [&](const float* dy, uint8_t* idx_or_null, float* dx) {
+        const bool host = i == p->rider_host && p->reduce_riders && defer && n_jobs > 0 && !side_jobs;
+        bool rode = false;
+        const int r = launch_conv_bwd_data(c, L, dy, idx_or_null, xmask, dx, host ? jobs : nullptr, n_jobs, &rode);
+        if (rode) { n_jobs = 0; ++p->rider_count; }
         return r;
     };
     if (L.vgg && L.pool22 && !L.bn && (L.wg & WG_3X3)) {
@@ -709,7 +743,7 @@
         if (wdone && !ddone && i > 0 && !L.drop && !L.extra_grad) {
             if (!gout_d) { gout_d = take(); gout_d_buf = taken; }
             probe_begin(1);
-            rc = launch_conv_bwd_data(c, L, gin, pidx, xmask, gout_d);
+            rc = bwd_data(gin, pidx, gout_d);
             if (rc == 0) { ddone = true; probe_end(1); }
             else if (rc != CLHIP_ENOTSUP) return rc;
         }
@@ -744,7 +778,7 @@
     float* gout = gout_d;
     if (gout) taken = gout_d_buf; else gout = take();
     probe_begin(1);
-    rc = launch_conv_bwd_data(c, L, gy, nullptr, xmask, gout);
+    rc = bwd_data(gy, nullptr, gout);
     if (rc) return rc;
     probe_end(1);
     gin = gout; gin_buf = taken;
@@ -846,6 +880,11 @@
     return p ? (int)(p->edge_count & 0x7fffffffu) : CLHIP_EINVAL;
 }
 
+int clhip_net_reduce_rider_count(void* handle) {
+    NetPlan* p = static_cast<NetPlan*>(handle);
+    return p ? (int)(p->rider_count & 0x7fffffffu) : CLHIP_EINVAL;
+}
+
 int clhip_net_prepared_weights(void* handle, size_t* ws_byte_off, size_t* bytes) {
     NetPlan* p = static_cast<NetPlan*>(handle);
     if (!p || !ws_byte_off || !bytes) return CLHIP_EINVAL;
diff --git a/clsurvey_amd/csrc/wgrad_reduce.hpp b/clsurvey_amd/csrc/wgrad_reduce.hpp
--- /dev/null
+++ b/clsurvey_amd/csrc/wgrad_reduce.hpp
@@ -0,0 +1,71 @@
+#pragma once
+#include "common.hpp"
+
+constexpr int RED_EL = 64, RED_J = 16, RED_V = 4;
+constexpr int RED_THREADS = RED_EL / RED_V * RED_J;
+
+template <int EL, int J>
+__device__ __forceinline__ void wgrad_reduce_block(const float* __restrict__ part, float* __restrict__ dw, float* __restrict__ db,
+                                                   int K, int C, int splits, size_t e0, double (*partial)[EL], int T = 9) {
+    const size_t kc = (size_t)K * C, nw = (size_t)T * kc, total = nw + K;
+    const int v = threadIdx.x % (EL / RED_V), j = threadIdx.x / (EL / RED_V);
+    const size_t e = e0 + (size_t)v * RED_V;
+    const int q = (splits + J - 1) / J;
+    const int s0 = j * q, s1 = min(splits, s0 + q);
+    double s[RED_V] = {0.0, 0.0, 0.0, 0.0};
+    if ((total & 3) == 0 && (reinterpret_cast<uintptr_t>(part) & 15u) == 0 && e + RED_V <= total) {
+#pragma unroll 4
+        for (int sp = s0; sp < s1; ++sp) {
+            const float4 t = *reinterpret_cast<const float4*>(part + (size_t)sp * total + e);
+            s[0] += (double)t.x; s[1] += (double)t.y; s[2] += (double)t.z; s[3] += (double)t.w;
+        }
+    } else {
+        for (int sp = s0; sp < s1; ++sp)
+#pragma unroll
+            for (int t = 0; t < RED_V; ++t)
+                if (e + t < total) s[t] += (double)part[(size_t)sp * total + e + t];
+    }
+#pragma unroll
+    for (int t = 0; t < RED_V; ++t) partial[j][v * RED_V + t] = s[t];
+    __syncthreads();
+    if (threadIdx.x < EL) {
+        const int el = threadIdx.x;
+        const size_t ee = e0 + el;
+        if (ee < total) {
+            double t = 0.0;
+#pragma unroll
+            for (int jj = 0; jj < J; ++jj) t += partial[jj][el];
+            if (ee < nw) {
+                const size_t rs = ee / kc, rem = ee - rs * kc;
+                dw[rem * T + rs] = (float)t;
+            } else if (db) {
+                db[ee - nw] = (float)t;
+            }
+        }
+    }
+}
+
+struct RedJobs {
+    clhip_wgrad_job job[CLHIP_WGRAD_JOBS_MAX];
+    unsigned first[CLHIP_WGRAD_JOBS_MAX + 1];
+    int n;
+};
+
+template <int EL, int JL>
+__device__ __forceinline__ void wgrad_reduce_unit(const RedJobs& jobs, unsigned u, double (*partial)[EL]) {
+    int ji = 0;
+    while (ji + 1 < jobs.n && u >= jobs.first[ji + 1]) ++ji;
+    const clhip_wgrad_job J = jobs.job[ji];
+    wgrad_reduce_block<EL, JL>(J.part, J.dw, J.db, J.K, J.C, J.splits, (size_t)(u - jobs.first[ji]) * EL, partial, J.taps ? J.taps : 9);
+}
+
+inline void wgrad_reduce_fill(RedJobs& r, const clhip_wgrad_job* jobs, int n) {
+    r.n = n;
+    r.first[0] = 0;
+    for (int i = 0; i < n; ++i) {
+        r.job[i] = jobs[i];
+        const size_t total = (size_t)(jobs[i].taps ? jobs[i].taps : 9) * jobs[i].K * jobs[i].C + jobs[i].K;
+        r.first[i + 1] = r.first[i] + (unsigned)((total + RED_EL - 1) / RED_EL);
+    }
+    for (int i = n; i < CLHIP_WGRAD_JOBS_MAX; ++i) { r.job[i] = clhip_wgrad_job{nullptr, nullptr, nullptr, 0, 0, 0, 0}; r.first[i + 1] = r.first[n]; }
+}
diff --git a/clsurvey_amd/net.py b/clsurvey_amd/net.py
--- a/clsurvey_amd/net.py
+++ b/clsurvey_amd/net.py
@@ -257,6 +257,12 @@
             raise RuntimeError("clhip_net_edge_grid_count")
         return n
 
+    def reduce_rider_count(self):
+        n = _lib.lib().clhip_net_reduce_rider_count(self._h)
+        if n < 0:
+            raise RuntimeError("clhip_net_reduce_rider_count")
+        return n
+
     def layer_paths(self, layer):
         bits = _lib.lib().clhip_net_layer_paths(self._h, int(layer))
         if bits < 0:
diff --git a/include/clhip.h b/include/clhip.h
--- a/include/clhip.h
+++ b/include/clhip.h
@@ -148,6 +148,15 @@
                          int H, int W, int relu, void* ws, size_t ws_bytes, void* stream);
 int clhip_conv3x3_bs_bwd_data(const float* dy, const uint8_t* idx_u8_or_null, const float* w, const float* relu_src, float* dx,
                               int N, int C, int K, int H, int W, void* ws, size_t ws_bytes, void* stream);
+typedef struct clhip_reduce_job {
+    const float* slabs;
+    float* dw;
+    float* db;
+    int K, C, splits, taps;
+} clhip_reduce_job;
+int clhip_conv3x3_bs_bwd_data_riders(const float* dy, const uint8_t* idx_u8_or_null, const float* w, const float* relu_src, float* dx,
+                                     int N, int C, int K, int H, int W, void* ws, size_t ws_bytes, const clhip_reduce_job* jobs,
+                                     int n_jobs, int place, int riders, void* stream);
 size_t clhip_conv5x5_bs_ws(int C, int K);
 int clhip_conv5x5_bs_fwd(const float* x, const float* w, const float* b, float* y, int N, int C, int K, int H, int W, int relu,
                          void* ws, size_t ws_bytes, void* stream);
@@ -228,6 +237,7 @@
 int clhip_net_layer_pool_idx(void* handle, int layer, size_t* ws_byte_off, size_t* elems_per_sample);
 int clhip_net_prepared_weights(void* handle, size_t* ws_byte_off, size_t* bytes);
 int clhip_net_edge_grid_count(void* handle);
+int clhip_net_reduce_rider_count(void* handle);
 int clhip_net_layer_paths(void* handle, int layer);
 
 int clhip_net_layer_input(void* handle, int layer, size_t* ws_float_off, size_t* in_elems);
```

New measurement: 307,600 images/s, median of 6. 1.01x the previous value.
